# nyu-systems/CLM-GS

Hardware: AMD Instinct MI355X
Metric: training images/s (Rubble-4K 28M Gaussians clm_offload) (higher is better)
Workload: dtype f32

## Files before the change

clm_gs_amd/_lib.py:

```python
import ctypes
import os
import time

import torch

_HERE = os.path.dirname(os.path.abspath(__file__))
LIB_PATH = os.environ.get("CLMGS_LIB_PATH") or os.path.join(_HERE, "libclmgs_hip.so")

_vp, _i, _i64, _f, _sz = ctypes.c_void_p, ctypes.c_int, ctypes.c_int64, ctypes.c_float, ctypes.c_size_t
_d = ctypes.c_double

SIGNATURES = {
    "clmgs_version": (_i, []),
    "clmgs_last_error": (ctypes.c_char_p, []),
    "clmgs_projection_fwd": (_i, [_vp, _i, _i, _vp, _vp, _vp, _vp, _vp, _i, _i, _f, _f, _f, _f, _vp, _vp, _vp, _vp]),
    "clmgs_visibility_select_temp_bytes": (_sz, [_i, _i]),
    "clmgs_visibility_select_count": (_i, [_vp, _i, _i, _vp, _vp, _vp, _vp, _vp, _i, _i, _f, _f, _f, _f, _vp, _sz, _vp]),
    "clmgs_visibility_select_count_blocks": (_i, [_vp, _i, _i, _vp, _vp, _vp, _vp, _vp, _i, _i, _f, _f, _f, _f, _vp, _sz, _vp, _vp]),
    "clmgs_visibility_select_emit": (_i, [_vp, _i, _i, _vp, _vp]),
    "clmgs_visibility_raw": (_i, [_vp, _i, _i, _vp, _vp, _vp, _vp, _vp, _i, _i, _f, _f, _f, _f, _vp]),
    "clmgs_projection_bwd": (_i, [_vp, _i, _i, _vp, _vp, _vp, _vp, _vp, _i, _i, _f, _vp, _vp, _vp, _vp, _vp, _vp, _vp]),
    "clmgs_sh_fwd": (_i, [_vp, _i, _i, _vp, _vp, _vp, _vp]),
    "clmgs_sh_bwd": (_i, [_vp, _i, _i, _vp, _vp, _vp, _vp, _vp, _i, _vp]),
    "clmgs_isect_count_temp_bytes": (_sz, [_i]),
    "clmgs_isect_count": (_i, [_vp, _i, _i, _vp, _vp, _i, _i, _i, _vp, _vp, _vp, _sz]),
    "clmgs_isect_sort_temp_bytes": (_sz, [_i64]),
    "clmgs_isect_emit_sort": (_i, [_vp, _i, _i, _i64, _vp, _vp, _vp, _vp, _i, _i, _i, _vp, _vp, _vp, _sz]),
    "clmgs_isect_offsets": (_i, [_vp, _i64, _vp, _i, _i, _i, _vp]),
    "clmgs_isect2_order_temp_bytes": (_sz, [_i]),
    "clmgs_isect2_order_count": (_i, [_vp, _i, _vp, _vp, _vp, _i, _i, _i, _vp, _vp, _vp, _vp, _vp, _vp, _sz, _vp]),
    "clmgs_isect2_sort_temp_bytes": (_sz, [_i64]),
    "clmgs_isect2_emit_sort": (_i, [_vp, _i, _i64, _vp, _vp, _vp, _vp, _i, _i, _vp, _vp, _vp, _vp, _vp, _sz, _vp]),
    "clmgs_isect2_emit_sort_dev": (_i, [_vp, _i, _i64, _vp, _vp, _vp, _vp, _vp, _i, _i, _vp, _vp, _vp, _vp, _vp, _sz, _vp]),
    "clmgs_isect3_front_temp_bytes": (_sz, [_i, _i]),
    "clmgs_isect3_front": (_i, [_vp, _i, _vp, _vp, _i, _i, _i, _vp, _vp, _vp, _vp, _sz]),
    "clmgs_isect3_bin_temp_bytes": (_sz, [_i64, _i]),
    "clmgs_isect3_bin": (_i, [_vp, _i, _i64, _vp, _i, _i, _vp, _vp, _vp, _vp, _vp, _vp, _vp, _sz]),
    "clmgs_isect3_bin_dev": (_i, [_vp, _i, _i64, _vp, _vp, _i, _i, _vp, _vp, _vp, _vp, _vp, _vp, _vp, _sz]),
    "clmgs_rasterize_fwd_dev": (_i, [_vp, _i, _i, _i64, _vp, _vp, _i, _i, _i, _i, _i, _vp, _vp, _vp, _vp, _vp, _vp]),
    "clmgs_rasterize_bwd_dev": (_i, [_vp, _i, _i, _i64, _vp, _vp, _vp, _i, _i, _i, _i, _i, _vp, _vp, _vp, _vp, _vp, _vp, _vp, _vp, _vp]),
    "clmgs_rasterize_pack_bytes": (_sz, [_i, _i]),
    "clmgs_rasterize_fwd": (_i, [_vp, _i, _i, _i64, _vp, _vp, _vp, _vp, _vp, _i, _i, _i, _i, _i, _vp, _vp, _vp, _vp, _vp, _vp]),
    "clmgs_rasterize_partials_bytes": (_sz, [_i64]),
    "clmgs_rasterize_bwd": (_i, [_vp, _i, _i, _i64, _vp, _vp, _i, _i, _i, _i, _i, _vp, _vp, _vp, _vp, _vp, _vp, _vp, _vp, _vp, _vp, _vp, _vp, _vp, _vp]),
    "clmgs_rasterize4_fwd": (_i, [_vp, _i, _i, _i64, _vp, _vp, _vp, _vp, _vp, _i, _i, _i, _i, _i, _vp, _vp, _vp, _vp, _vp, _vp]),
    "clmgs_rasterize4_bwd": (_i, [_vp, _i, _i, _i64, _vp, _vp, _i, _i, _i, _i, _i, _vp, _vp, _vp, _vp, _vp, _vp, _vp, _vp, _vp, _vp, _vp, _vp, _vp, _vp]),
    "clmgs_rasterize4_slot_bwd": (_i, [_vp, _i, _i, _i64, _vp, _vp, _i, _i, _i, _i, _i, _vp, _vp, _vp, _vp, _vp, _vp, _vp, _vp, _vp, _vp, _vp, _vp, _vp, _vp]),
    "clmgs_rasterize4_fwd_dev": (_i, [_vp, _i, _i, _i64, _vp, _vp, _i, _i, _i, _i, _i, _vp, _vp, _vp, _vp, _vp, _vp]),
    "clmgs_rasterize4_bwd_dev": (_i, [_vp, _i, _i, _i64, _vp, _vp, _vp, _i, _i, _i, _i, _i, _vp, _vp, _vp, _vp, _vp, _vp, _vp, _vp, _vp]),
    "clmgs_preprocess_fwd": (_i, [_vp, _i, _vp, _vp, _vp, _vp, _vp, _vp, _i, _vp, _vp, _vp, _i, _i, _i, _f, _f, _f, _f, _vp, _vp, _vp, _vp, _vp, _vp, _vp, _vp]),
    "clmgs_preprocess_bwd": (_i, [_vp, _i, _vp, _vp, _vp, _vp, _vp, _vp, _i, _vp, _vp, _vp, _i, _i, _i, _f, _vp, _vp, _vp, _vp, _vp, _vp, _vp, _vp, _vp, _vp, _vp, _i, _vp, _vp, _vp, _vp, _i]),
    "clmgs_rasterize_abs_bwd": (_i, [_vp, _i, _i, _i64, _vp, _vp, _i, _i, _i, _i, _i, _vp, _vp, _vp, _vp, _vp, _vp, _vp, _vp, _vp, _vp, _vp, _vp, _vp, _vp, _vp]),
    "clmgs_rasterize_abs_bwd_dev": (_i, [_vp, _i, _i, _i64, _vp, _vp, _vp, _i, _i, _i, _i, _i, _vp, _vp, _vp, _vp, _vp, _vp, _vp, _vp, _vp]),
    "clmgs_preprocess_abs_bwd": (_i, [_vp, _i, _vp, _vp, _vp, _vp, _vp, _vp, _i, _vp, _vp, _vp, _i, _i, _i, _f, _vp, _vp, _vp, _vp, _vp, _vp, _vp, _vp, _vp, _vp, _vp, _i, _vp, _vp, _vp, _vp, _i, _vp]),
    "clmgs_projection_aa_fwd": (_i, [_vp, _i, _i, _vp, _vp, _vp, _vp, _vp, _i, _i, _f, _f, _f, _f, _vp, _vp, _vp, _vp, _vp]),
    "clmgs_projection_aa_bwd": (_i, [_vp, _i, _i, _vp, _vp, _vp, _vp, _vp, _i, _i, _f, _vp, _vp, _vp, _vp, _vp, _vp, _vp, _vp]),
    "clmgs_preprocess_aa_fwd": (_i, [_vp, _i, _vp, _vp, _vp, _vp, _vp, _vp, _i, _vp, _vp, _vp, _i, _i, _i, _f, _f, _f, _f, _vp, _vp, _vp, _vp, _vp, _vp, _vp, _vp]),
    "clmgs_preprocess_aa_bwd": (_i, [_vp, _i, _vp, _vp, _vp, _vp, _vp, _vp, _i, _vp, _vp, _vp, _i, _i, _i, _f, _vp, _vp, _vp, _vp, _vp, _vp, _vp, _vp, _vp, _vp, _vp, _i, _vp, _vp, _vp, _vp, _i]),
    "clmgs_preprocess_aa_abs_bwd": (_i, [_vp, _i, _vp, _vp, _vp, _vp, _vp, _vp, _i, _vp, _vp, _vp, _i, _i, _i, _f, _vp, _vp, _vp, _vp, _vp, _vp, _vp, _vp, _vp, _vp, _vp, _i, _vp, _vp, _vp, _vp, _i, _vp]),
    "clmgs_ssim_fwd": (_i, [_vp, _i, _i, _i, _i, _vp, _vp, _vp, _vp, _vp, _vp]),
    "clmgs_ssim_bwd": (_i, [_vp, _i, _i, _i, _i, _vp, _vp, _vp, _f, _vp, _vp, _vp, _vp]),
    "clmgs_loss_slots": (_i, []),
    "clmgs_l1_ssim_loss_fwd": (_i, [_vp, _i, _i, _vp, _i64, _i64, _i64, _vp, _vp, _vp, _vp, _vp]),
    "clmgs_l1_ssim_loss_bwd": (_i, [_vp, _i, _i, _vp, _i64, _i64, _i64, _vp, _vp, _f, _vp, _vp, _vp, _vp]),
    "clmgs_l1_ssim_loss_masked_fwd": (_i, [_vp, _i, _i, _vp, _i64, _i64, _i64, _vp, _vp, _vp, _vp, _vp, _vp]),
    "clmgs_l1_ssim_loss_masked_bwd": (_i, [_vp, _i, _i, _vp, _i64, _i64, _i64, _vp, _vp, _f, _vp, _vp, _vp, _vp, _vp]),
    "clmgs_exposure_partials_rows": (_i, [_i, _i]),
    "clmgs_exposure_fwd": (_i, [_vp, _i, _i, _vp, _i64, _i64, _i64, _vp, _vp, _i64, _i64, _i64]),
    "clmgs_exposure_bwd": (_i, [_vp, _i, _i, _vp, _i64, _i64, _i64, _vp, _vp, _i64, _i64, _i64, _vp, _i64, _i64, _i64, _vp]),
    "clmgs_exposure_grad_finish": (_i, [_vp, _i, _vp, _vp]),
    "clmgs_invdepth_partials_rows": (_i, [_i, _i]),
    "clmgs_invdepth_pack": (_i, [_vp, _i, _vp, _vp, _vp]),
    "clmgs_invdepth_l1_fwd_bwd": (_i, [_vp, _i, _i, _vp, _i64, _i64, _vp, _f, _f, _vp, _f, _vp, _i64, _i64, _vp]),
    "clmgs_invdepth_finish": (_i, [_vp, _i, _vp, _vp]),
    "clmgs_invdepth_rows_bwd": (_i, [_vp, _i, _vp, _vp, _vp, _vp, _vp, _vp, _vp, _vp, _i]),
    "clmgs_mcmc_relocation": (_i, [_vp, _i64, _vp, _vp, _vp, _vp, _vp]),
    "clmgs_mcmc_reg_grad": (_i, [_vp, _i64, _vp, _i64, _vp, _i64, _vp, _i64, _vp, _i64, _f, _f]),
    "clmgs_mcmc_noise": (_i, [_vp, _i64, _vp, _vp, _vp, _vp, _vp, _f, _vp]),
    "clmgs_rows_gather": (_i, [_vp, _vp, _vp, _vp, _vp, _i, _i64, _i, _i]),
    "clmgs_rows_scatter_add": (_i, [_vp, _vp, _vp, _vp, _vp, _i, _i64, _i, _i]),
    "clmgs_scatter_to_bit": (_i, [_vp, _vp, _i, _vp, _i64, _i]),
    "clmgs_extract_ffs": (_i, [_vp, _vp, _i, _i64, _vp]),
    "clmgs_pair_overlap_count": (_i, [_vp, _vp, _i, _i64, _i, _vp]),
    "clmgs_set_signal": (_i, [_vp, _vp, _i, ctypes.c_int32]),
    "clmgs_adam_rows": (_i, [_vp, _vp, _vp, _vp, _vp, _vp, _i, _vp, _i64, _i, _vp, _d, _d, _d, _i, _i, _f, _i]),
    "clmgs_pack_small": (_i, [_vp, _i64, _vp, _vp, _vp, _vp, _vp]),
    "clmgs_adam_small_packed": (_i, [_vp, _i64, _vp, _vp, _vp, _vp, _vp, _vp, _d, _d, _d, _i, _i, _f, _vp, _i]),
    "clmgs_adam_catch_up": (_i, [_vp, _vp, _vp, _vp, _vp, _vp, _i, _i64, _i, _vp, _d, _d, _d, _i, _i, _i, _vp, _vp, _f, _i]),
    "clmgs_host_adam_rows": (_i, [_vp, _vp, _vp, _vp, _vp, _i64, _i, _vp, _d, _d, _d, _i, _i, _f, _i, _vp, _i]),
    "clmgs_host_pool_start": (_i, [_i]),
    "clmgs_host_usable_cpus": (_i, []),
    "clmgs_memcpy_async": (_i, [_vp, _vp, _vp, _sz, _i]),
    "clmgs_host_rows_prepare": (_i, [_vp, _vp, _vp, _vp, _vp, _vp, _vp, _i64, _i, _vp, _d, _d, _d, _i, _i, _i, _f, _i, _vp, _i]),
    "clmgs_densify_stats": (_i, [_vp, _i64, _vp, _vp, _vp, _i, _f, _f, _vp, _vp, _vp]),
    "clmgs_morton_order_temp_bytes": (_sz, [_i64]),
    "clmgs_morton_order": (_i, [_vp, _i64, _vp, _vp, _vp, _vp, _sz]),
    "clmgs_tsp_tour": (_i, [_i, _vp, _vp]),
    "clmgs_knn3_mean_dist2": (_i, [_vp, _i, _vp, _vp, _f, _f, _f, _f, _i, _i, _i, _i, _vp]),
    "clmgs_host_groups_temp_bytes": (_sz, [_i64]),
    "clmgs_host_groups": (_i, [_vp, _i64, _vp, _vp, _i, _i, _vp, _i, _vp, _vp, _vp, _vp, _vp, _sz]),
    "clmgs_publish_pack": (_i, [_vp, _vp, _vp, _vp, _vp, _i, _i64, _i64, _i64, _i]),
    "clmgs_visibility_candidates": (_i, [_vp, _i, _i, _i, _i, _vp, _vp, _vp, _vp, _i, _i, _f, _f, _f, _f, _f, _vp]),
    "clmgs_small_rows_scatter": (_i, [_vp, _i64, _vp, _vp, _vp, _vp, _vp, _vp, _vp]),
    "clmgs_adam_small_packed_range": (_i, [_vp, _i64, _i64, _i64, _vp, _vp, _vp, _vp, _vp, _vp, _d, _d, _d, _i, _i, _f, _vp, _i]),
    "clmgs_small_deferred_kmax": (_i, []),
    "clmgs_adam_small_deferred": (_i, [_vp, _i64, _vp, _vp, _vp, _vp, _vp, _vp, _vp, _i, _i, _vp, _vp, _vp, _vp, _d, _d, _d,
                                       _f, _i, _vp, _vp, _i, _i, _f, _f, _f, _i, _vp]),
    "clmgs_device_errors": (_i, [_vp, _i]),
    "clmgs_pinned_alloc": (_vp, [_sz]),
    "clmgs_pinned_free": (_i, [_vp]),
}

_lib = None

TIMING = None
STATS = {"n_isects": [], "n_emitted": [], "host_wait_s": 0.0}


class ClmgsError(RuntimeError):
    pass


class _Entry:

    def __init__(self, name, fn, takes_stream):
        self.name, self.fn, self.takes_stream = name, fn, takes_stream

    def __call__(self, *args):
        if TIMING is None or not self.takes_stream:
            return self.fn(*args)
        s, e = torch.cuda.Event(enable_timing=True), torch.cuda.Event(enable_timing=True)
        h = getattr(args[0], "value", args[0])
        st = torch.cuda.ExternalStream(h) if h else torch.cuda.current_stream()
        s.record(st)
        rc = self.fn(*args)
        e.record(st)
        TIMING.setdefault(self.name, []).append((s, e))
        return rc


class _Namespace:
    pass


_NO_STREAM = {"clmgs_version", "clmgs_loss_slots", "clmgs_exposure_partials_rows", "clmgs_invdepth_partials_rows", "clmgs_small_deferred_kmax", "clmgs_isect3_front_temp_bytes",
              "clmgs_isect3_bin_temp_bytes", "clmgs_last_error", "clmgs_isect_count_temp_bytes",
              "clmgs_isect_sort_temp_bytes", "clmgs_host_groups_temp_bytes", "clmgs_isect2_order_temp_bytes", "clmgs_isect2_sort_temp_bytes", "clmgs_visibility_select_temp_bytes", "clmgs_rasterize_pack_bytes", "clmgs_rasterize_partials_bytes", "clmgs_host_adam_rows", "clmgs_host_pool_start", "clmgs_host_usable_cpus", "clmgs_host_rows_prepare", "clmgs_tsp_tour",
              "clmgs_pinned_alloc", "clmgs_pinned_free", "clmgs_device_errors"}


def timing_summary():
    out = {}
    for name, evs in (TIMING or {}).items():
        out[name] = (len(evs), sum(s.elapsed_time(e) for s, e in evs))
    return out


def lib():
    global _lib
    if _lib is None:
        if not os.path.exists(LIB_PATH):
            raise ClmgsError(
                f"{LIB_PATH} not found: build it with `python -c 'import __graft_entry__ as g; g.build()'` "
                "(make -C clm_gs_amd/csrc).  clm_gs_amd has no CPU/eager fallback."
            )
        l = ctypes.CDLL(LIB_PATH)
        ns = _Namespace()
        for name, (res, args) in SIGNATURES.items():
            fn = getattr(l, name)
            fn.restype = res
            fn.argtypes = args
            setattr(ns, name, _Entry(name, fn, name not in _NO_STREAM))
        _lib = ns
    return _lib


def check(rc):
    if rc != 0:
        msg = lib().clmgs_last_error()
        raise ClmgsError(f"libclmgs_hip error {rc}: {msg.decode() if msg else ''}")


def check_device_errors():
    bits = ctypes.c_uint32(0)
    check(lib().clmgs_device_errors(ctypes.byref(bits), 1))
    if bits.value & 4:
        raise ClmgsError("deferred small-attribute Adam: a block of rows was further behind than the recorded step history "
                         "(clmgs_adam_small_deferred, device error bit 4): its parameters are wrong")
    if bits.value:
        raise ClmgsError(f"device error word {bits.value}: no kernel of this library raises that value (4 is the only one "
# ... 68 lines not shown
```

clm_gs_amd/csrc/clm_ops.hip:

```cpp
#include <stdlib.h>

#include "common.h"
#include "vis_math.h"
#include "radix.h"

namespace clmgs {
__device__ uint32_t g_dev_err;
static uint32_t* device_error_word() {
  static thread_local uint32_t* p[16] = {nullptr};
  int dev = 0;
  if (hipGetDevice(&dev) != hipSuccess || dev < 0 || dev >= 16) dev = 0;
  if (!p[dev]) {
    void* a = nullptr;
    if (hipGetSymbolAddress(&a, HIP_SYMBOL(g_dev_err)) == hipSuccess) p[dev] = (uint32_t*)a;
  }
  return p[dev];
}


template <typename IdxT>
__device__ __forceinline__ int64_t row_of(const void* idx, int64_t i) {
  return idx ? (int64_t)reinterpret_cast<const IdxT*>(idx)[i] : i;
}

// ... 426 lines not shown
        int row[4];
#pragma unroll
        for (int k = 0; k < 4; ++k) {
          row[k] = (i + k) / w;
          gg[k] = sg[row[k] * 12 + co + (i + k - row[k] * w)] * grad_scale;
        }
        step(ti, row, pp, mm, vv, gg);
#pragma unroll
        for (int k = 0; k < 4; ++k) sp[row[k] * 12 + co + (i + k - row[k] * w)] = pp[k];
        *reinterpret_cast<float4*>(P + i) = make_float4(pp[0], pp[1], pp[2], pp[3]);
        *reinterpret_cast<float4*>(M + i) = make_float4(mm[0], mm[1], mm[2], mm[3]);
        *reinterpret_cast<float4*>(V + i) = make_float4(vv[0], vv[1], vv[2], vv[3]);
      } else {
        for (int idx = i; idx < n_el; ++idx) {
          const int row[1] = {idx / w};
          float pp[1] = {P[idx]}, mm[1] = {M[idx]}, vv[1] = {V[idx]};
          const float gg[1] = {sg[row[0] * 12 + co + (idx - row[0] * w)] * grad_scale};
          step(ti, row, pp, mm, vv, gg);
          P[idx] = pp[0]; M[idx] = mm[0]; V[idx] = vv[0];
          sp[row[0] * 12 + co + (idx - row[0] * w)] = pp[0];
        }
      }
    }
  }
  __syncthreads();
}

template <bool RANGE>
__global__ void __launch_bounds__(SA_ROWS)
adam_small_packed_kernel(int64_t n, int64_t row_begin, int64_t row_end, SmallAdam t, float4* __restrict__ packed_p,
                         float4* __restrict__ packed_g, float beta1, float beta2, float ob1,
                         float ob2, float eps, float inv_bc1, float inv_sqrt_bc2, float grad_scale,
                         const int32_t* __restrict__ g_stamp, int cur_step) {
  __shared__ __attribute__((aligned(16))) float sg[SA_ROWS * 12];
  __shared__ __attribute__((aligned(16))) float sp[SA_ROWS * 12];
  const int tid = threadIdx.x;
  const int64_t n_blocks = RANGE ? (row_end + SA_ROWS - 1) / SA_ROWS : (n + SA_ROWS - 1) / SA_ROWS;
  for (int64_t blk = (RANGE ? row_begin / SA_ROWS : 0) + blockIdx.x; blk < n_blocks; blk += gridDim.x) {
    const int64_t row0 = blk * SA_ROWS;
    const int rows = (int)min((int64_t)SA_ROWS, n - row0);
    __syncthreads();
    if (g_stamp) {
      __shared__ uint8_t has_g[SA_ROWS];
      if (tid < rows) has_g[tid] = (uint8_t)(g_stamp[row0 + tid] == cur_step);
      __syncthreads();
      small_stage(sg, packed_g, row0, rows, [&](int row) { return has_g[row] != 0; });
    } else {
      small_stage(sg, packed_g, row0, rows, [](int) { return true; });
    }
    small_walk(t, row0, rows, sg, sp, grad_scale,
               [&](int ti, const auto& row, auto& pp, auto& mm, auto& vv, const auto& gg) {
      const float lr_bc = t.lr[ti] * inv_bc1;
      constexpr int N = (int)(sizeof(pp) / sizeof(float));
      float pn[N], m2[N], v2[N];
#pragma unroll
      for (int k = 0; k < N; ++k) {
        m2[k] = mm[k]; v2[k] = vv[k];
        pn[k] = adam_elem(m2[k], v2[k], pp[k], gg[k], lr_bc, beta1, beta2, ob1, ob2, eps, inv_sqrt_bc2);
      }
#pragma unroll
      for (int k = 0; k < N; ++k) {
        const bool act = !RANGE || (row0 + row[k] >= row_begin && row0 + row[k] < row_end);
        pp[k] = act ? pn[k] : pp[k]; mm[k] = act ? m2[k] : mm[k]; vv[k] = act ? v2[k] : vv[k];
      }
    });
    const float4 z = make_float4(0.f, 0.f, 0.f, 0.f);
    for (int i = tid; i < rows * 3; i += SA_ROWS) {
      packed_p[row0 * 3 + i] = reinterpret_cast<const float4*>(sp)[i];
      const float4 gq = reinterpret_cast<const float4*>(sg)[i];
      if (!g_stamp && (gq.x != 0.f || gq.y != 0.f || gq.z != 0.f || gq.w != 0.f))
        packed_g[row0 * 3 + i] = z;
    }
  }
}

constexpr int SD_KMAX = 16;
struct SmallDeferred {
  float lr[SD_KMAX][4];
  float inv_bc1[SD_KMAX], inv_sqrt_bc2[SD_KMAX];
  float pos_margin[SD_KMAX + 1], scale_gain[SD_KMAX + 1];
  int to_step;
};

__global__ void __launch_bounds__(SA_ROWS)
adam_small_deferred_kernel(int64_t n, SmallAdam t, float4* __restrict__ packed_p, const float4* __restrict__ packed_g,
                           const int32_t* __restrict__ g_stamp, int32_t* __restrict__ blk_last, SmallDeferred d,
                           float beta1, float beta2, float ob1, float ob2, float eps, float grad_scale, int C,
                           const float* __restrict__ viewmats, const float* __restrict__ Ks, float W, float H, float eps2d,
                           float near_plane, float far_plane, int flush_all, uint8_t* __restrict__ blk_flag, int n_hist,
                           uint32_t* __restrict__ dev_err) {
  __shared__ __attribute__((aligned(16))) float sg[SA_ROWS * 12];
  __shared__ __attribute__((aligned(16))) float sp[SA_ROWS * 12];
  __shared__ int gstep_s[SA_ROWS];
  __shared__ float cam_s[VB_MAX_CAMS][VB_CAM_F];
  const int tid = threadIdx.x;
  if (!flush_all) {
    for (int c = tid; c < C; c += SA_ROWS) vis_store_cam(cam_s[c], viewmats + 16 * c, Ks + 9 * c, W, H);
  }
  const float near_m = near_plane - (fabsf(near_plane) * 1e-5f + 1e-6f);
  const float far_m = far_plane + fabsf(far_plane) * 1e-5f;
  const int64_t n_blocks = (n + SA_ROWS - 1) / SA_ROWS;
  for (int64_t blk = blockIdx.x; blk < n_blocks; blk += gridDim.x) {
    const int last = blk_last[blk];
    int k = d.to_step - last;
    if (k <= 0 && (flush_all || !blk_flag)) continue;
    if (k > n_hist) {
      if (tid == 0 && dev_err) atomicOr(dev_err, 4u);
      k = n_hist;
    }
    const int64_t row0 = blk * SA_ROWS;
    const int rows = (int)min((int64_t)SA_ROWS, n - row0);
    __syncthreads();
    if (!flush_all) {
      const int kk = min(max(k, 0), SD_KMAX);
      bool cand = false;
      if (tid < rows) {
        const float* x = t.p[0] + 3 * (row0 + tid);
        const float* ls = t.p[2] + 3 * (row0 + tid);
        const float m[3] = {x[0], x[1], x[2]};
        const float sgn = __expf(fmaxf(ls[0], fmaxf(ls[1], ls[2]))) * d.scale_gain[kk];
        const float smax2g = sgn * sgn;
        cand = !(smax2g < 1e30f);
        for (int c = 0; c < C && !cand; ++c)
          cand = vis_candidate(lds_cam(cam_s[c]), cam_s[c][16], m, smax2g, d.pos_margin[kk], W, H, eps2d, near_m, far_m);
      }
      const bool any = __syncthreads_or(cand);
      if (blk_flag && tid == 0) blk_flag[blk] = any ? 1 : 0;
      if (k <= 0 || (!any && k < SD_KMAX)) continue;
    }
    if (tid < rows) {
      const int gs = g_stamp[row0 + tid];
      gstep_s[tid] = (gs > last && gs <= d.to_step) ? gs : -1;
    }
    __syncthreads();
    small_stage(sg, packed_g, row0, rows, [&](int row) { return gstep_s[row] >= 0; });
    small_walk(t, row0, rows, sg, sp, grad_scale,
               [&](int ti, const auto& row, auto& pp, auto& mm, auto& vv, const auto& gg) {
      constexpr int N = (int)(sizeof(pp) / sizeof(float));
      int gst[N];
#pragma unroll
      for (int q = 0; q < N; ++q) gst[q] = gstep_s[row[q]];
      for (int s_ = last + 1; s_ <= d.to_step; ++s_) {
        const int j = d.to_step - s_;
        const float lr_bc = d.lr[j][ti] * d.inv_bc1[j];
        const float isb2 = d.inv_sqrt_bc2[j];
#pragma unroll
        for (int q = 0; q < N; ++q)
          pp[q] = adam_elem(mm[q], vv[q], pp[q], gst[q] == s_ ? gg[q] : 0.f, lr_bc, beta1, beta2, ob1, ob2, eps, isb2);
      }
    });
    for (int i = tid; i < rows * 3; i += SA_ROWS) packed_p[row0 * 3 + i] = reinterpret_cast<const float4*>(sp)[i];
    if (tid == 0) blk_last[blk] = d.to_step;
  }
}

__global__ void __launch_bounds__(256)
pack_small_kernel(int64_t n, const float* __restrict__ xyz, const float* __restrict__ opa,
                  const float* __restrict__ sca, const float* __restrict__ rot,
                  float4* __restrict__ packed_p) {
  for (int64_t r = blockIdx.x * (int64_t)blockDim.x + threadIdx.x; r < n;
       r += (int64_t)gridDim.x * blockDim.x) {
    const float4 q = *reinterpret_cast<const float4*>(rot + 4 * r);
    packed_p[3 * r] = make_float4(xyz[3 * r], xyz[3 * r + 1], xyz[3 * r + 2], opa[r]);
    packed_p[3 * r + 1] = make_float4(sca[3 * r], sca[3 * r + 1], sca[3 * r + 2], q.x);
    packed_p[3 * r + 2] = make_float4(q.y, q.z, q.w, 0.f);
  }
}

__global__ void __launch_bounds__(256)
small_rows_scatter_kernel(int64_t n_rows, const int64_t* __restrict__ rows, const float4* __restrict__ src,
                          float* __restrict__ xyz, float* __restrict__ opa, float* __restrict__ sca,
                          float* __restrict__ rot, float4* __restrict__ packed_p) {
  for (int64_t i = blockIdx.x * (int64_t)blockDim.x + threadIdx.x; i < n_rows;
       i += (int64_t)gridDim.x * blockDim.x) {
    const int64_t r = rows[i];
    const float4 a = src[3 * i], b = src[3 * i + 1], c = src[3 * i + 2];
    xyz[3 * r] = a.x; xyz[3 * r + 1] = a.y; xyz[3 * r + 2] = a.z;
    opa[r] = a.w;
    sca[3 * r] = b.x; sca[3 * r + 1] = b.y; sca[3 * r + 2] = b.z;
    *reinterpret_cast<float4*>(rot + 4 * r) = make_float4(b.w, c.x, c.y, c.z);
    packed_p[3 * r] = a; packed_p[3 * r + 1] = b; packed_p[3 * r + 2] = make_float4(c.x, c.y, c.z, 0.f);
  }
}

__global__ void __launch_bounds__(256)
densify_stats_kernel(int64_t n, const int64_t* __restrict__ filter,
                     const float* __restrict__ v_means2d, const int32_t* __restrict__ radii,
                     int only_visible, float half_w, float half_h, float* __restrict__ max_radii2D,
                     float* __restrict__ accum, float* __restrict__ denom) {
  for (int64_t i = blockIdx.x * (int64_t)blockDim.x + threadIdx.x; i < n;
       i += (int64_t)gridDim.x * blockDim.x) {
    const int r = radii[i];
    if (only_visible && r <= 0) continue;
    const int64_t g = filter ? filter[i] : i;
    const float gx = v_means2d[2 * i] * half_w, gy = v_means2d[2 * i + 1] * half_h;
    max_radii2D[g] = fmaxf(max_radii2D[g], (float)r);
    accum[g] += sqrtf(gx * gx + gy * gy);
    denom[g] += 1.f;
  }
}

}

using namespace clmgs;

extern "C" int clmgs_rows_gather(void* stream, float* dst, const float* src, const void* dst_idx,
                                 const void* src_idx, int idx_is_64, int64_t n_rows, int cols,
                                 int grid_blocks) {
  return rows_move<false>(stream, dst, src, dst_idx, src_idx, idx_is_64, n_rows, cols, grid_blocks);
}

extern "C" int clmgs_publish_pack(void* stream, float* msg, const float* table, const int64_t* own_rows,
                                  const int32_t* stamp, int step, int64_t lo, int64_t n_rows, int64_t chunk,
                                  int cols) {
  CLMGS_CHECK_ARG(n_rows >= 0 && chunk >= n_rows && cols > 0 && cols % 4 == 0);
  if (n_rows == 0) return 0;
  CLMGS_CHECK_ARG(msg && table && own_rows && (((uintptr_t)msg | (uintptr_t)table) & 15) == 0);
  const int64_t total = n_rows * (cols / 4);
  hipLaunchKernelGGL(publish_pack_kernel, dim3(min(ceil_div(total, 256), 256 * 8)), dim3(256), 0, (hipStream_t)stream,
                     msg, table, own_rows, stamp, step, lo, n_rows, chunk, cols / 4);
  CLMGS_LAUNCH_CHECK();
  return 0;
}

extern "C" int clmgs_rows_scatter_add(void* stream, float* dst, const float* src,
                                      const void* dst_idx, const void* src_idx, int idx_is_64,
                                      int64_t n_rows, int cols, int grid_blocks) {
  return rows_move<true>(stream, dst, src, dst_idx, src_idx, idx_is_64, n_rows, cols, grid_blocks);
}

#define DISPATCH_ELEM(bytes, CALL)                    \
  switch (bytes) {                                    \
    case 1: { typedef int8_t T; CALL; } break;        \
    case 2: { typedef int16_t T; CALL; } break;       \
    case 4: { typedef int32_t T; CALL; } break;       \
// ... 224 lines not shown
                     (float)(1.0 - beta1), (float)(1.0 - beta2), keep_grad)
  if (idx_is_64) { if (v4) CLMGS_CATCH_UP(int64_t, 4); else CLMGS_CATCH_UP(int64_t, 1); }
  else { if (v4) CLMGS_CATCH_UP(int32_t, 4); else CLMGS_CATCH_UP(int32_t, 1); }
#undef CLMGS_CATCH_UP
  CLMGS_LAUNCH_CHECK();
  return 0;
}

extern "C" int clmgs_pack_small(void* stream, int64_t n, const float* xyz, const float* opacity,
                                const float* scaling, const float* rotation, void* packed_p) {
  CLMGS_CHECK_ARG(n >= 0);
  if (n == 0) return 0;
  CLMGS_CHECK_ARG(xyz && opacity && scaling && rotation && packed_p && (((uintptr_t)packed_p & 15) == 0));
  hipLaunchKernelGGL(pack_small_kernel, dim3(min(ceil_div(n, 256), 256 * 16)), dim3(256), 0,
                     (hipStream_t)stream, n, xyz, opacity, scaling, rotation, (float4*)packed_p);
  CLMGS_LAUNCH_CHECK();
  return 0;
}

extern "C" int clmgs_small_rows_scatter(void* stream, int64_t n_rows, const int64_t* rows, const void* lines,
                                        float* xyz, float* opacity, float* scaling, float* rotation,
                                        void* packed_p) {
  CLMGS_CHECK_ARG(n_rows >= 0);
  if (n_rows == 0) return 0;
  CLMGS_CHECK_ARG(rows && lines && xyz && opacity && scaling && rotation && packed_p &&
                  (((uintptr_t)packed_p | (uintptr_t)lines | (uintptr_t)rotation) & 15) == 0);
  hipLaunchKernelGGL(small_rows_scatter_kernel, dim3(min(ceil_div(n_rows, 256), 256 * 16)), dim3(256), 0,
                     (hipStream_t)stream, n_rows, rows, (const float4*)lines, xyz, opacity, scaling, rotation,
                     (float4*)packed_p);
  CLMGS_LAUNCH_CHECK();
  return 0;
}

extern "C" int clmgs_adam_small_packed_range(void* stream, int64_t n, int64_t row_begin, int64_t row_end,
                                             float* const* params, float* const* exp_avg,
                                             float* const* exp_avg_sq, const double* lr4, void* packed_p,
                                             void* packed_g, double beta1, double beta2, double eps, int step,
                                             int bias_correction, float grad_scale, const int32_t* g_stamp,
                                             int cur_step);

extern "C" int clmgs_adam_small_packed(void* stream, int64_t n, float* const* params,
                                       float* const* exp_avg, float* const* exp_avg_sq,
                                       const double* lr4, void* packed_p, void* packed_g,
                                       double beta1, double beta2, double eps, int step,
                                       int bias_correction, float grad_scale, const int32_t* g_stamp,
                                       int cur_step) {
  return clmgs_adam_small_packed_range(stream, n, 0, -1, params, exp_avg, exp_avg_sq, lr4, packed_p, packed_g, beta1,
                                       beta2, eps, step, bias_correction, grad_scale, g_stamp, cur_step);
}

extern "C" int clmgs_adam_small_packed_range(void* stream, int64_t n, int64_t row_begin, int64_t row_end,
                                             float* const* params, float* const* exp_avg,
                                             float* const* exp_avg_sq, const double* lr4, void* packed_p,
                                             void* packed_g, double beta1, double beta2, double eps, int step,
                                             int bias_correction, float grad_scale, const int32_t* g_stamp,
                                             int cur_step) {
  CLMGS_CHECK_ARG(n >= 0 && step >= 1);
  const bool ranged = row_end >= 0;
  if (ranged) CLMGS_CHECK_ARG(row_begin >= 0 && row_begin <= row_end && row_end <= n);
  if (n == 0 || (ranged && row_end == row_begin)) return 0;
  CLMGS_CHECK_ARG(lr4 && packed_p && packed_g && (((uintptr_t)packed_p | (uintptr_t)packed_g) & 15) == 0);
  SmallAdam t;
  CLMGS_CHECK_ARG(small_adam_fill(&t, params, exp_avg, exp_avg_sq, lr4));
  float inv_bc1, inv_sqrt_bc2;
  adam_bias_host(beta1, beta2, step, bias_correction, &inv_bc1, &inv_sqrt_bc2);
  const float ob1 = (float)(1.0 - beta1), ob2 = (float)(1.0 - beta2);
  if (ranged) {
    const int64_t blocks = (row_end + SA_ROWS - 1) / SA_ROWS - row_begin / SA_ROWS;
    hipLaunchKernelGGL(adam_small_packed_kernel<true>, dim3(min(blocks, (int64_t)256 * 16)), dim3(SA_ROWS), 0,
                       (hipStream_t)stream, n, row_begin, row_end, t, (float4*)packed_p, (float4*)packed_g,
                       (float)beta1, (float)beta2, ob1, ob2, (float)eps, inv_bc1, inv_sqrt_bc2, grad_scale, g_stamp,
                       cur_step);
  } else {
    hipLaunchKernelGGL(adam_small_packed_kernel<false>, dim3(min(ceil_div(n, SA_ROWS), 256 * 16)), dim3(SA_ROWS), 0,
                       (hipStream_t)stream, n, (int64_t)0, n, t, (float4*)packed_p, (float4*)packed_g, (float)beta1,
                       (float)beta2, ob1, ob2, (float)eps, inv_bc1, inv_sqrt_bc2, grad_scale, g_stamp, cur_step);
  }
  CLMGS_LAUNCH_CHECK();
  return 0;
}

extern "C" int clmgs_small_deferred_kmax(void) { return SD_KMAX; }

extern "C" int clmgs_adam_small_deferred(void* stream, int64_t n, float* const* params, float* const* exp_avg,
                                         float* const* exp_avg_sq, void* packed_p, const void* packed_g,
                                         const int32_t* g_stamp, int32_t* blk_last, int to_step, int n_hist,
                                         const double* lr4_hist, const int32_t* step_index, const float* pos_margin,
                                         const float* scale_gain, double beta1, double beta2, double eps,
                                         float grad_scale, int C, const float* viewmats, const float* Ks, int width,
                                         int height, float eps2d, float near_plane, float far_plane, int flush_all,
                                         uint8_t* blk_flag) {
  CLMGS_CHECK_ARG(n >= 0 && to_step >= 0 && n_hist >= 0 && n_hist <= SD_KMAX);
  CLMGS_CHECK_ARG(!blk_flag || !flush_all);
  if (n == 0) return 0;
  if (n_hist == 0) {
    if (blk_flag) CLMGS_HIP(hipMemsetAsync(blk_flag, 1, (size_t)((n + SA_ROWS - 1) / SA_ROWS), (hipStream_t)stream));
    return 0;
  }
  CLMGS_CHECK_ARG(packed_p && packed_g && g_stamp && blk_last && lr4_hist && step_index && pos_margin && scale_gain &&
                  (((uintptr_t)packed_p | (uintptr_t)packed_g) & 15) == 0);
  CLMGS_CHECK_ARG(flush_all || (C >= 1 && C <= VB_MAX_CAMS && viewmats && Ks && width > 0 && height > 0));
  SmallAdam t;
  CLMGS_CHECK_ARG(small_adam_fill(&t, params, exp_avg, exp_avg_sq, nullptr));
  SmallDeferred d;
  for (int j = 0; j < SD_KMAX; ++j) {
    const int jj = j < n_hist ? j : n_hist - 1;
    for (int i = 0; i < 4; ++i) d.lr[j][i] = (float)lr4_hist[4 * jj + i];
    CLMGS_CHECK_ARG(step_index[jj] >= 1);
    adam_bias_host(beta1, beta2, step_index[jj], 1, &d.inv_bc1[j], &d.inv_sqrt_bc2[j]);
  }
  for (int k = 0; k <= SD_KMAX; ++k) {
    const int kk = k <= n_hist ? k : n_hist;
    d.pos_margin[k] = pos_margin[kk];
    d.scale_gain[k] = scale_gain[kk];
  }
  d.to_step = to_step;
  const float ob1 = (float)(1.0 - beta1), ob2 = (float)(1.0 - beta2);
  hipLaunchKernelGGL(adam_small_deferred_kernel, dim3(min(ceil_div(n, SA_ROWS), 256 * 16)), dim3(SA_ROWS), 0,
                     (hipStream_t)stream, n, t, (float4*)packed_p, (const float4*)packed_g, g_stamp, blk_last, d,
                     (float)beta1, (float)beta2, ob1, ob2, (float)eps, grad_scale, C, viewmats, Ks, (float)width,
                     (float)height, eps2d, near_plane, far_plane, flush_all, blk_flag, n_hist, device_error_word());
  CLMGS_LAUNCH_CHECK();
  return 0;
}

extern "C" int clmgs_device_errors(uint32_t* out, int reset) {
  CLMGS_CHECK_ARG(out);
  CLMGS_HIP(hipDeviceSynchronize());
  CLMGS_HIP(hipMemcpyFromSymbol(out, HIP_SYMBOL(clmgs::g_dev_err), sizeof(uint32_t)));
  if (reset && *out) {
    const uint32_t z = 0;
    CLMGS_HIP(hipMemcpyToSymbol(HIP_SYMBOL(clmgs::g_dev_err), &z, sizeof(z)));
  }
  return 0;
}

extern "C" int clmgs_densify_stats(void* stream, int64_t n, const int64_t* filter,
                                   const float* v_means2d, const int32_t* radii,
                                   int only_visible, float half_w, float half_h,
                                   float* max_radii2D, float* xyz_gradient_accum,
                                   float* denom) {
  CLMGS_CHECK_ARG(n >= 0);
  if (n == 0) return 0;
  CLMGS_CHECK_ARG(v_means2d && radii && max_radii2D && xyz_gradient_accum && denom);
  const int grid = min(ceil_div(n, 256), 256 * 8);
  hipLaunchKernelGGL(densify_stats_kernel, dim3(grid), dim3(256), 0, (hipStream_t)stream, n, filter,
                     v_means2d, radii, only_visible, half_w, half_h, max_radii2D,
                     xyz_gradient_accum, denom);
  CLMGS_LAUNCH_CHECK();
  return 0;
}
```

clm_gs_amd/csrc/isect.hip:

```cpp
#include <stdlib.h>

#include "common.h"
#include "gs_math.h"
#include "radix.h"
#include "vis_math.h"
#include "isect_math.h"

namespace clmgs {

__global__ void __launch_bounds__(256)
isect_count_kernel(int64_t CN, const float* __restrict__ means2d, const int32_t* __restrict__ radii,
                   float tile_size, int tile_w, int tile_h, int32_t* __restrict__ tiles_per_gauss,
                   int64_t* __restrict__ cum) {
  for (int64_t i = blockIdx.x * (int64_t)blockDim.x + threadIdx.x; i < CN;
       i += (int64_t)gridDim.x * blockDim.x) {
    int cnt = 0;
    const int r = radii[i];
    if (r > 0) {
      const float2 m = *reinterpret_cast<const float2*>(means2d + 2 * i);
      const TileBox b = tile_box(m.x, m.y, (float)r, tile_size, tile_w, tile_h);
      cnt = (b.x1 - b.x0) * (b.y1 - b.y0);
    }
    tiles_per_gauss[i] = cnt;
    cum[i] = cnt;
// ... 431 lines not shown
}

extern "C" size_t clmgs_isect2_sort_temp_bytes(int64_t n_isects) {
  if (n_isects <= 0) return 256;
  return 6 * align_up((size_t)n_isects * 4, 256) + radix_table_bytes(n_isects) + 256;
}

static int isect2_emit_sort_impl(void* stream, int V, int64_t n_isects, const float* depths,
                                 const int32_t* order, const int64_t* cum,
                                 const uint64_t* boxes, int tile_width, int tile_height,
                                 int32_t* flatten_ids, int32_t* offsets, int64_t* isect_ids,
                                 int32_t* emit_slot, void* temp, size_t temp_bytes,
                                 const int64_t* row_cum, const int64_t* n_dev) {
  CLMGS_CHECK_ARG(V >= 0 && n_isects >= 0 && offsets);
  hipStream_t s = (hipStream_t)stream;
  const int n_tiles = tile_width * tile_height;
  if (n_isects == 0) {
    CLMGS_HIP(hipMemsetAsync(offsets, 0, sizeof(int32_t) * (size_t)n_tiles, s));
    return 0;
  }
  CLMGS_CHECK_ARG(n_isects < ((int64_t)1 << 31));
  CLMGS_CHECK_ARG(depths && order && cum && boxes && flatten_ids && temp);
  CLMGS_CHECK_ARG(temp_bytes >= clmgs_isect2_sort_temp_bytes(n_isects));
  char* base = (char*)temp;
  const size_t a4 = align_up((size_t)n_isects * 4, 256);
  uint32_t* k_a = (uint32_t*)base; base += a4;
  uint32_t* k_b = (uint32_t*)base; base += a4;
  char* v_a = base; base += 2 * a4;
  char* v_b = base; base += 2 * a4;
  uint32_t* table = (uint32_t*)base;
  const bool slots = emit_slot != nullptr;
  CLMGS_CHECK_ARG(!slots || row_cum);
  const int tile_bits = ilog2_floor((unsigned)n_tiles) + 1;
  const int n_blocks = (int)((n_isects + RS_MIN_CHUNK - 1) / RS_MIN_CHUNK);
  if (slots)
    hipLaunchKernelGGL((isect2_emit_hist_kernel<true>), dim3(n_blocks), dim3(256), 0, s, V, n_isects, n_dev, order,
                       (const unsigned long long*)boxes, cum, tile_width, row_cum, k_a, (int32_t*)nullptr, (int2*)v_a,
                       n_blocks, table);
  else
    hipLaunchKernelGGL((isect2_emit_hist_kernel<false>), dim3(n_blocks), dim3(256), 0, s, V, n_isects, n_dev, order,
                       (const unsigned long long*)boxes, cum, tile_width, row_cum, k_a, (int32_t*)v_a, (int2*)nullptr,
                       n_blocks, table);
  CLMGS_LAUNCH_CHECK();
  uint32_t* sorted = nullptr;
  int rc;
  if (slots)
    rc = radix_sort_pairs_impl<uint32_t, int2, RS_DEFAULT_ITEMS>(s, n_isects, k_a, k_b, (int2*)v_a, (int2*)v_b, (int2*)nullptr,
                                                                  0, tile_bits, table, &sorted, n_dev, flatten_ids, emit_slot,
                                                                  true);
  else
    rc = radix_sort_pairs_impl<uint32_t, int32_t, RS_DEFAULT_ITEMS>(s, n_isects, k_a, k_b, (int32_t*)v_a, (int32_t*)v_b,
                                                                     flatten_ids, 0, tile_bits, table, &sorted, n_dev,
                                                                     nullptr, nullptr, true);
  if (rc) return rc;
  hipLaunchKernelGGL(isect2_offsets_kernel, dim3(min(ceil_div(n_isects, 256), 256 * 16)), dim3(256), 0, s,
                     n_isects, sorted, n_tiles, offsets, flatten_ids, depths, isect_ids, n_dev);
  CLMGS_LAUNCH_CHECK();
  return 0;
}

extern "C" int clmgs_isect2_emit_sort(void* stream, int V, int64_t n_isects, const float* depths,
                                      const int32_t* order, const int64_t* cum,
                                      const uint64_t* boxes, int tile_width, int tile_height,
                                      int32_t* flatten_ids, int32_t* offsets, int64_t* isect_ids,
                                      int32_t* emit_slot, void* temp, size_t temp_bytes,
                                      const int64_t* row_cum) {
  return isect2_emit_sort_impl(stream, V, n_isects, depths, order, cum, boxes, tile_width, tile_height,
                               flatten_ids, offsets, isect_ids, emit_slot, temp, temp_bytes, row_cum, nullptr);
}

extern "C" int clmgs_isect2_emit_sort_dev(void* stream, int V, int64_t capacity, const int64_t* n_isects_dev,
                                          const float* depths, const int32_t* order, const int64_t* cum,
                                          const uint64_t* boxes, int tile_width, int tile_height,
                                          int32_t* flatten_ids, int32_t* offsets, int64_t* isect_ids,
                                          int32_t* emit_slot, void* temp, size_t temp_bytes,
                                          const int64_t* row_cum) {
  CLMGS_CHECK_ARG(n_isects_dev && capacity > 0);
  return isect2_emit_sort_impl(stream, V, capacity, depths, order, cum, boxes, tile_width, tile_height,
                               flatten_ids, offsets, isect_ids, emit_slot, temp, temp_bytes, row_cum, n_isects_dev);
}

namespace clmgs {

constexpr int VB_CH = 4;

__device__ __forceinline__ int vis_classify(const Cam& c, float kc, const float m[3], float smax2,
                                            float W, float H, float eps2d, float near_m, float far_m,
                                            float near_p, float far_p, bool accept_ok) {
  const float x = c.R[0] * m[0] + c.R[1] * m[1] + c.R[2] * m[2] + c.t[0];
  const float y = c.R[3] * m[0] + c.R[4] * m[1] + c.R[5] * m[2] + c.t[1];
  const float z = c.R[6] * m[0] + c.R[7] * m[1] + c.R[8] * m[2] + c.t[2];
  if (z < near_m || z > far_m) return 0;
  const float rz = __builtin_amdgcn_rcpf(z);
  const float mx = c.fx * x * rz + c.cx, my = c.fy * y * rz + c.cy;
  const float B = smax2 * rz * rz * kc + eps2d;
  if (accept_ok && z > near_p && z < far_p && B < 400.f && mx >= 1.f && mx <= W - 1.f && my >= 1.f &&
      my <= H - 1.f)
    return 1;
  const float Rb = 3.03f * __builtin_amdgcn_sqrtf(2.f * B + 0.1f) + 2.f;
  return (mx + Rb <= 0.f || mx - Rb >= W || my + Rb <= 0.f || my - Rb >= H) ? 0 : 2;
}

__global__ void __launch_bounds__(256)
visibility_bits_kernel(int C, int N, int W64, const float* __restrict__ means,
                       const float* __restrict__ quats_raw, const float* __restrict__ log_scales,
                       const float* __restrict__ viewmats, const float* __restrict__ Ks, float W, float H,
                       float eps2d, float near_plane, float far_plane, float radius_clip,
                       unsigned long long* __restrict__ bits, int64_t* __restrict__ counts,
                       const uint8_t* __restrict__ blk_flag) {
  __shared__ float cam_s[VB_MAX_CAMS][VB_CAM_F];
  __shared__ float row_s[256][10];
  __shared__ unsigned short cand[256 * VB_CH];
  __shared__ int n_cand;
  __shared__ unsigned long long wb[VB_CH][4];
  __shared__ unsigned long long anyw[4];
  const int tid = threadIdx.x, lane = tid & 63;
  const unsigned long long lt = (1ull << lane) - 1ull;
  const float near_m = near_plane - (fabsf(near_plane) * 1e-5f + 1e-6f);
  const float far_m = far_plane + fabsf(far_plane) * 1e-5f;
  const float near_p = near_plane + (fabsf(near_plane) * 1e-5f + 1e-6f);
  const float far_p = far_plane - fabsf(far_plane) * 1e-5f;
  const bool accept_ok = radius_clip < 1.5f && eps2d >= 0.3f;
  const int wid = tid >> 6;
  for (int c = tid; c < C; c += 256) {
    const Cam cam = load_cam(viewmats + 16 * c, Ks + 9 * c);
    float* f = cam_s[c];
    for (int i = 0; i < 9; ++i) f[i] = cam.R[i];
    f[9] = cam.t[0]; f[10] = cam.t[1]; f[11] = cam.t[2];
    f[12] = cam.fx; f[13] = cam.fy; f[14] = cam.cx; f[15] = cam.cy;
    f[16] = vis_cam_kc(cam, W, H);
  }
  const int n_rb = (W64 + 3) / 4;
  float nm0 = 0.f, nm1 = 0.f, nm2 = 0.f, nl0 = 0.f, nl1 = 0.f, nl2 = 0.f;
  float4 nq = make_float4(0.f, 0.f, 0.f, 0.f);
  auto fetch = [&](int rbn) {
    const int n = rbn * 256 + tid;
    const bool live_n = rbn < n_rb && (!blk_flag || blk_flag[rbn]);
    const int nn = (live_n && n < N) ? n : 0;
    nm0 = means[3 * nn]; nm1 = means[3 * nn + 1]; nm2 = means[3 * nn + 2];
    nq = *reinterpret_cast<const float4*>(quats_raw + 4 * nn);
    nl0 = log_scales[3 * nn]; nl1 = log_scales[3 * nn + 1]; nl2 = log_scales[3 * nn + 2];
  };
  fetch(blockIdx.x);
  for (int rb = blockIdx.x; rb < n_rb; rb += gridDim.x) {
    const int n = rb * 256 + tid;
    const bool in = n < N;
    const float m[3] = {nm0, nm1, nm2};
    const float4 q4 = nq;
    const float s0 = __expf(nl0), s1 = __expf(nl1), s2 = __expf(nl2);
    fetch(rb + gridDim.x);
    if (blk_flag && !blk_flag[rb]) {
      if (tid < (C + 1) * 4) {
        const int c = tid >> 2, w = rb * 4 + (tid & 3);
        if (w < W64) { bits[(size_t)c * W64 + w] = 0ull; counts[(size_t)c * W64 + w] = 0; }
      }
      for (int q = tid + 256; q < (C + 1) * 4; q += 256) {
        const int c = q >> 2, w = rb * 4 + (q & 3);
        if (w < W64) { bits[(size_t)c * W64 + w] = 0ull; counts[(size_t)c * W64 + w] = 0; }
      }
      continue;
    }
    const float smax = fmaxf(s0, fmaxf(s1, s2));
    const float smax2 = smax * smax;
    const float qn2 = q4.x * q4.x + q4.y * q4.y + q4.z * q4.z + q4.w * q4.w;
    const bool row_ok = accept_ok && qn2 >= 1e-20f && qn2 <= 1e20f && (s0 + s1 + s2) < 1e30f;
    lds_barrier();
    {
      float* r = row_s[tid];
      r[0] = m[0]; r[1] = m[1]; r[2] = m[2]; r[3] = q4.x; r[4] = q4.y; r[5] = q4.z; r[6] = q4.w;
      r[7] = s0; r[8] = s1; r[9] = s2;
    }
    if (tid < 4) anyw[tid] = 0ull;
    for (int c0 = 0; c0 < C; c0 += VB_CH) {
      const int cn = min(VB_CH, C - c0);
      if (tid < VB_CH * 4) wb[tid >> 2][tid & 3] = 0ull;
      if (tid == 0) n_cand = 0;
      lds_barrier();
      for (int cc = 0; cc < cn; ++cc) {
        const Cam cam = load_cam(viewmats + 16 * (c0 + cc), Ks + 9 * (c0 + cc));
        const int cls = in ? vis_classify(cam, cam_s[c0 + cc][16], m, smax2, W, H, eps2d, near_m, far_m,
                                          near_p, far_p, row_ok) : 0;
        const unsigned long long acc = __ballot(cls == 1);
        if (lane == 0 && acc) atomicOr(&wb[cc][wid], acc);
        const bool pass = cls == 2;
        const unsigned long long b = __ballot(pass);
        int base = 0;
        if (lane == 0 && b) base = atomicAdd(&n_cand, __popcll(b));
        base = __builtin_amdgcn_readfirstlane(base);
        if (pass) cand[base + __popcll(b & lt)] = (unsigned short)(tid | (cc << 8));
      }
      lds_barrier();
      const int nc = n_cand;
      for (int k = tid; k < nc; k += 256) {
        const int e = cand[k], r = e & 255, cc = e >> 8;
        const Cam cam = lds_cam(cam_s[c0 + cc]);
        const float* rr = row_s[r];
        const float mm[3] = {rr[0], rr[1], rr[2]};
        const float qq[4] = {rr[3], rr[4], rr[5], rr[6]};
        const float ss[3] = {rr[7], rr[8], rr[9]};
        const Proj p = project_fwd(cam, mm, qq, ss, W, H, eps2d, near_plane, far_plane, radius_clip);
        if (p.radius > 0) atomicOr(&wb[cc][r >> 6], 1ull << (r & 63));
      }
      lds_barrier();
      if (tid < cn * 4) {
        const int cc = tid >> 2, j = tid & 3, w = rb * 4 + j;
        if (w < W64) {
          const unsigned long long b = wb[cc][j];
          bits[(size_t)(c0 + cc) * W64 + w] = b;
          counts[(size_t)(c0 + cc) * W64 + w] = __popcll(b);
          if (b) atomicOr(&anyw[j], b);
        }
      }
    }
    lds_barrier();
    if (tid < 4 && rb * 4 + tid < W64) {
      bits[(size_t)C * W64 + rb * 4 + tid] = anyw[tid];
      counts[(size_t)C * W64 + rb * 4 + tid] = __popcll(anyw[tid]);
    }
  }
}

__global__ void __launch_bounds__(256)
visibility_candidates_kernel(int C, int N, int own_lo, int own_hi, const float* __restrict__ means,
                             const float* __restrict__ log_scales, const float* __restrict__ viewmats,
                             const float* __restrict__ Ks, float W, float H, float eps2d, float near_plane,
                             float far_plane, float pos_margin, float scale_gain, uint8_t* __restrict__ mask) {
  __shared__ float cam_s[VB_MAX_CAMS][VB_CAM_F];
  const int tid = threadIdx.x;
  for (int c = tid; c < C; c += 256) {
    const Cam cam = load_cam(viewmats + 16 * c, Ks + 9 * c);
    float* f = cam_s[c];
    for (int i = 0; i < 9; ++i) f[i] = cam.R[i];
    f[9] = cam.t[0]; f[10] = cam.t[1]; f[11] = cam.t[2];
    f[12] = cam.fx; f[13] = cam.fy; f[14] = cam.cx; f[15] = cam.cy;
    f[16] = vis_cam_kc(cam, W, H);
  }
  __syncthreads();
  const float near_m = near_plane - (fabsf(near_plane) * 1e-5f + 1e-6f);
  const float far_m = far_plane + fabsf(far_plane) * 1e-5f;
  for (int n = blockIdx.x * 256 + tid; n < N; n += gridDim.x * 256) {
    if (n >= own_lo && n < own_hi) {
      mask[n] = 0;
      continue;
    }
    const float m[3] = {means[3 * n], means[3 * n + 1], means[3 * n + 2]};
    const float lmax = fmaxf(log_scales[3 * n], fmaxf(log_scales[3 * n + 1], log_scales[3 * n + 2]));
    const float sg = __expf(lmax) * scale_gain;
    const float smax2g = sg * sg;
    bool any = !(smax2g < 1e30f);
    for (int c = 0; c < C && !any; ++c)
      any = vis_candidate(lds_cam(cam_s[c]), cam_s[c][16], m, smax2g, pos_margin, W, H, eps2d, near_m, far_m);
    mask[n] = any ? 1 : 0;
  }
}

__global__ void __launch_bounds__(256)
visibility_emit_kernel(int C, int N, int W64, const unsigned long long* __restrict__ bits,
                       const int64_t* __restrict__ scan, int64_t* __restrict__ out) {
  const int64_t total = (int64_t)(C + 1) * W64 * 64;
  for (int64_t t = blockIdx.x * (int64_t)blockDim.x + threadIdx.x; t < total;
       t += (int64_t)gridDim.x * blockDim.x) {
    const int64_t word = t >> 6;
    const int bit = (int)(t & 63);
    const unsigned long long b = bits[word];
    if ((b >> bit) & 1ull) {
      const int64_t end = scan[word];
      const int64_t pos = end - __popcll(b) + __popcll(b & ((1ull << bit) - 1ull));
      const int w = (int)(word % W64);
      out[pos] = (int64_t)w * 64 + bit;
    }
  }
}

}

extern "C" size_t clmgs_visibility_select_temp_bytes(int C, int N) {
  const size_t words = (size_t)(C + 1) * (size_t)((N + 63) / 64);
  return 2 * align_up(words * 8, 256) + scan_scratch_bytes((int64_t)words) + 256;
}

extern "C" int clmgs_visibility_select_count_blocks(void* stream, int C, int N, const float* means,
                                                    const float* quats_raw, const float* log_scales,
                                                    const float* viewmats, const float* Ks, int width, int height,
                                                    float eps2d, float near_plane, float far_plane,
                                                    float radius_clip, void* temp, size_t temp_bytes,
                                                    int64_t* cum_totals, const uint8_t* block_flags);

extern "C" int clmgs_visibility_select_count(void* stream, int C, int N, const float* means,
                                             const float* quats_raw, const float* log_scales,
                                             const float* viewmats, const float* Ks, int width,
                                             int height, float eps2d, float near_plane,
                                             float far_plane, float radius_clip, void* temp,
                                             size_t temp_bytes, int64_t* cum_totals) {
  return clmgs_visibility_select_count_blocks(stream, C, N, means, quats_raw, log_scales, viewmats, Ks, width, height,
                                              eps2d, near_plane, far_plane, radius_clip, temp, temp_bytes, cum_totals,
                                              nullptr);
}

extern "C" int clmgs_visibility_select_count_blocks(void* stream, int C, int N, const float* means,
                                                    const float* quats_raw, const float* log_scales,
                                                    const float* viewmats, const float* Ks, int width, int height,
                                                    float eps2d, float near_plane, float far_plane,
                                                    float radius_clip, void* temp, size_t temp_bytes,
                                                    int64_t* cum_totals, const uint8_t* block_flags) {
  CLMGS_CHECK_ARG(C >= 1 && C <= 64 && N >= 1 && width > 0 && height > 0);
  CLMGS_CHECK_ARG(means && quats_raw && log_scales && viewmats && Ks && temp && cum_totals);
  CLMGS_CHECK_ARG(temp_bytes >= clmgs_visibility_select_temp_bytes(C, N));
  hipStream_t s = (hipStream_t)stream;
  const int W64 = (N + 63) / 64;
  const size_t words = (size_t)(C + 1) * W64;
  char* base = (char*)temp;
  unsigned long long* bits = (unsigned long long*)base; base += align_up(words * 8, 256);
  int64_t* counts = (int64_t*)base; base += align_up(words * 8, 256);
  int64_t* scratch = (int64_t*)base;
  hipLaunchKernelGGL(visibility_bits_kernel, dim3(min(ceil_div((int64_t)W64 * 64, 256), 256 * 8)),
                     dim3(256), 0, s, C, N, W64, means, quats_raw, log_scales, viewmats, Ks,
                     (float)width, (float)height, eps2d, near_plane, far_plane, radius_clip, bits, counts, block_flags);
  CLMGS_LAUNCH_CHECK();
  const int rc = inclusive_scan_i64(s, (int64_t)words, counts, scratch);
  if (rc) return rc;
  for (int r = 0; r <= C; ++r)
    CLMGS_HIP(hipMemcpyAsync(cum_totals + r, counts + (size_t)(r + 1) * W64 - 1, sizeof(int64_t),
                             hipMemcpyDeviceToDevice, s));
  return 0;
}

extern "C" int clmgs_visibility_select_emit(void* stream, int C, int N, const void* temp,
                                            int64_t* out) {
  CLMGS_CHECK_ARG(C >= 1 && N >= 1 && temp && out);
  const int W64 = (N + 63) / 64;
  const size_t words = (size_t)(C + 1) * W64;
  const char* base = (const char*)temp;
  const unsigned long long* bits = (const unsigned long long*)base; base += align_up(words * 8, 256);
  const int64_t* scan = (const int64_t*)base;
  hipLaunchKernelGGL(visibility_emit_kernel, dim3(min(ceil_div((int64_t)words * 64, 256), 256 * 32)),
                     dim3(256), 0, (hipStream_t)stream, C, N, W64, bits, scan, out);
  CLMGS_LAUNCH_CHECK();
  return 0;
}


extern "C" int clmgs_visibility_candidates(void* stream, int C, int N, int own_lo, int own_hi, const float* means,
                                           const float* log_scales, const float* viewmats, const float* Ks,
                                           int width, int height, float eps2d, float near_plane, float far_plane,
                                           float pos_margin, float scale_gain, uint8_t* mask) {
  CLMGS_CHECK_ARG(C >= 1 && C <= 64 && N >= 1 && width > 0 && height > 0);
  CLMGS_CHECK_ARG(means && log_scales && viewmats && Ks && mask);
  CLMGS_CHECK_ARG(pos_margin >= 0.f && scale_gain >= 1.f && own_lo >= 0 && own_hi >= own_lo);
  hipLaunchKernelGGL(visibility_candidates_kernel, dim3(min(ceil_div((int64_t)N, 256), 256 * 16)), dim3(256), 0,
                     (hipStream_t)stream, C, N, own_lo, own_hi, means, log_scales, viewmats, Ks, (float)width,
                     (float)height, eps2d, near_plane, far_plane, pos_margin, scale_gain, mask);
  CLMGS_LAUNCH_CHECK();
  return 0;
}
```

clm_gs_amd/csrc/vis_math.h:

```cpp
#pragma once
#include "common.h"
#include "gs_math.h"

namespace clmgs {

constexpr int VB_CAM_F = 20;
constexpr int VB_MAX_CAMS = 64;

__device__ __forceinline__ float vis_cam_kc(const Cam& c, float W, float H) {
  const float tan_fovx = 0.5f * W / c.fx, tan_fovy = 0.5f * H / c.fy;
  const float limx = fmaxf(fabsf((W - c.cx) / c.fx), fabsf(c.cx / c.fx)) + 0.3f * tan_fovx;
  const float limy = fmaxf(fabsf((H - c.cy) / c.fy), fabsf(c.cy / c.fy)) + 0.3f * tan_fovy;
  return 0.505f * (c.fx * c.fx * (1.f + limx * limx) + c.fy * c.fy * (1.f + limy * limy));
}

__device__ __forceinline__ Cam lds_cam(const float* f) {
  Cam c;
#pragma unroll
  for (int i = 0; i < 9; ++i) c.R[i] = f[i];
  c.t[0] = f[9]; c.t[1] = f[10]; c.t[2] = f[11];
  c.fx = f[12]; c.fy = f[13]; c.cx = f[14]; c.cy = f[15];
  return c;
}


__device__ __forceinline__ bool vis_candidate(const Cam& c, float kc, const float m[3], float smax2g, float d,
                                              float W, float H, float eps2d, float near_m, float far_m) {
  const float x = c.R[0] * m[0] + c.R[1] * m[1] + c.R[2] * m[2] + c.t[0];
  const float y = c.R[3] * m[0] + c.R[4] * m[1] + c.R[5] * m[2] + c.t[1];
  const float z = c.R[6] * m[0] + c.R[7] * m[1] + c.R[8] * m[2] + c.t[2];
  const float zl = z - d, zh = z + d;
  if (zh < near_m || zl > far_m) return false;
  const float zc = fmaxf(fmaxf(zl, near_m), 1e-12f), zf = fmaxf(fminf(zh, far_m), zc);
  const float rzc = 1.f / zc, rzf = 1.f / zf;
  const float xh = x + d, xl = x - d, yh = y + d, yl = y - d;
  const float tx_max = xh > 0.f ? xh * rzc : xh * rzf, tx_min = xl < 0.f ? xl * rzc : xl * rzf;
  const float ty_max = yh > 0.f ? yh * rzc : yh * rzf, ty_min = yl < 0.f ? yl * rzc : yl * rzf;
  const float B = smax2g * rzc * rzc * kc + eps2d;
  const float Rb = 1.001f * (3.03f * sqrtf(2.f * B + 0.1f) + 2.f) + 1.f;
  const float mx_max = c.fx * tx_max + c.cx, mx_min = c.fx * tx_min + c.cx;
  const float my_max = c.fy * ty_max + c.cy, my_min = c.fy * ty_min + c.cy;
  return !(mx_max + Rb <= 0.f || mx_min - Rb >= W || my_max + Rb <= 0.f || my_min - Rb >= H);
}


__device__ __forceinline__ void vis_store_cam(float* f, const float* viewmat, const float* K, float W, float H) {
  const Cam cam = load_cam(viewmat, K);
  for (int i = 0; i < 9; ++i) f[i] = cam.R[i];
  f[9] = cam.t[0]; f[10] = cam.t[1]; f[11] = cam.t[2];
  f[12] = cam.fx; f[13] = cam.fy; f[14] = cam.cx; f[15] = cam.cy;
  f[16] = vis_cam_kc(cam, W, H);
}

}
```

clm_gs_amd/gsplat.py:

```python

import time

import torch

from . import _lib
from ._lib import check, dptr, stream

F32, I32, I64 = torch.float32, torch.int32, torch.int64


class _Projection(torch.autograd.Function):
    @staticmethod
    def forward(ctx, means, quats, scales, viewmats, Ks, width, height, eps2d, near_plane,
                far_plane, radius_clip):
        L = _lib.lib()
        means, quats, scales = means.contiguous(), quats.contiguous(), scales.contiguous()
        viewmats, Ks = viewmats.contiguous(), Ks.contiguous()
        C, N = viewmats.shape[0], means.shape[0]
        dev = means.device
        radii = torch.empty((C, N), dtype=I32, device=dev)
        means2d = torch.empty((C, N, 2), dtype=F32, device=dev)
        depths = torch.empty((C, N), dtype=F32, device=dev)
        conics = torch.empty((C, N, 3), dtype=F32, device=dev)
        check(L.clmgs_projection_fwd(
# ... 50 lines not shown
            float(near_plane), float(far_plane), float(radius_clip), dptr(radii), dptr(means2d),
            dptr(depths), dptr(conics), dptr(comps)))
        ctx.save_for_backward(means, quats, scales, viewmats, Ks, radii)
        ctx.cfg = (int(width), int(height), float(eps2d))
        ctx.mark_non_differentiable(radii)
        return radii, means2d, depths, conics, comps

    @staticmethod
    def backward(ctx, _v_radii, v_means2d, v_depths, v_conics, v_comps):
        L = _lib.lib()
        means, quats, scales, viewmats, Ks, radii = ctx.saved_tensors
        width, height, eps2d = ctx.cfg
        C, N = radii.shape
        dev = means.device
        if v_means2d is None:
            v_means2d = torch.zeros((C, N, 2), dtype=F32, device=dev)
        if v_conics is None:
            v_conics = torch.zeros((C, N, 3), dtype=F32, device=dev)
        v_means2d, v_conics = v_means2d.contiguous(), v_conics.contiguous()
        v_depths = v_depths.contiguous() if v_depths is not None else None
        v_comps = v_comps.contiguous() if v_comps is not None else None
        v_means = torch.empty_like(means)
        v_quats = torch.empty_like(quats)
        v_scales = torch.empty_like(scales)
        check(L.clmgs_projection_aa_bwd(
            stream(), C, N, dptr(means), dptr(quats), dptr(scales), dptr(viewmats), dptr(Ks),
            width, height, eps2d, dptr(radii), dptr(v_means2d, F32), dptr(v_depths, F32, True),
            dptr(v_conics, F32), dptr(v_comps, F32, True), dptr(v_means), dptr(v_quats), dptr(v_scales)))
        return v_means, v_quats, v_scales, None, None, None, None, None, None, None, None


def fully_fused_projection(means, covars, quats, scales, viewmats, Ks, width, height, eps2d=0.3,
                           near_plane=0.01, far_plane=1e10, radius_clip=0.0, packed=False,
                           sparse_grad=False, calc_compensations=False):
    if covars is not None:
        raise NotImplementedError("the CLM-GS engines always pass covars=None")
    if calc_compensations:
        if not packed:
            return _ProjectionAA.apply(means, quats, scales, viewmats, Ks, width, height, eps2d, near_plane,
                                       far_plane, radius_clip)
        with torch.no_grad():
            radii, means2d, depths, conics, comps = _ProjectionAA.apply(
                means, quats, scales, viewmats, Ks, width, height, eps2d, near_plane, far_plane, radius_clip)
            camera_ids, gaussian_ids = torch.nonzero(radii > 0, as_tuple=True)
            return (camera_ids, gaussian_ids, radii[camera_ids, gaussian_ids],
                    means2d[camera_ids, gaussian_ids], depths[camera_ids, gaussian_ids],
                    conics[camera_ids, gaussian_ids], comps[camera_ids, gaussian_ids])
    if not packed:
        radii, means2d, depths, conics = _Projection.apply(
            means, quats, scales, viewmats, Ks, width, height, eps2d, near_plane, far_plane,
            radius_clip)
        return radii, means2d, depths, conics, None
    with torch.no_grad():
        radii, means2d, depths, conics = _Projection.apply(
            means, quats, scales, viewmats, Ks, width, height, eps2d, near_plane, far_plane,
            radius_clip)
        camera_ids, gaussian_ids = torch.nonzero(radii > 0, as_tuple=True)
        return (camera_ids, gaussian_ids, radii[camera_ids, gaussian_ids],
                means2d[camera_ids, gaussian_ids], depths[camera_ids, gaussian_ids],
                conics[camera_ids, gaussian_ids], None)


def visibility_radii(means, quats, scales, viewmats, Ks, width, height, eps2d=0.3,
                     near_plane=0.01, far_plane=1e10, radius_clip=0.0, raw=False):
    L = _lib.lib()
    means, quats, scales = means.contiguous(), quats.contiguous(), scales.contiguous()
    viewmats, Ks = viewmats.contiguous(), Ks.contiguous()
    C, N = viewmats.shape[0], means.shape[0]
    radii = torch.empty((C, N), dtype=I32, device=means.device)
    if raw:
        check(L.clmgs_visibility_raw(
            stream(), C, N, dptr(means, F32), dptr(quats, F32), dptr(scales, F32), dptr(viewmats, F32),
            dptr(Ks, F32), int(width), int(height), float(eps2d), float(near_plane), float(far_plane),
            float(radius_clip), dptr(radii)))
        return radii
    check(L.clmgs_projection_fwd(
        stream(), C, N, dptr(means, F32), dptr(quats, F32), dptr(scales, F32), dptr(viewmats, F32),
        dptr(Ks, F32), int(width), int(height), float(eps2d), float(near_plane), float(far_plane),
        float(radius_clip), dptr(radii), None, None, None))
    return radii


def visibility_select(means, quats_raw, log_scales, viewmats, Ks, width, height, eps2d=0.3,
                      near_plane=0.01, far_plane=1e10, radius_clip=0.0, block_flags=None):
    L = _lib.lib()
    means, quats_raw, log_scales = means.contiguous(), quats_raw.contiguous(), log_scales.contiguous()
    viewmats, Ks = viewmats.contiguous(), Ks.contiguous()
    C, N = viewmats.shape[0], means.shape[0]
    dev = means.device
    tb = L.clmgs_visibility_select_temp_bytes(C, N)
    temp = torch.empty((tb,), dtype=torch.uint8, device=dev)
    cum = torch.empty((C + 1,), dtype=I64, device=dev)
    check(L.clmgs_visibility_select_count_blocks(
        stream(), C, N, dptr(means, F32), dptr(quats_raw, F32), dptr(log_scales, F32), dptr(viewmats, F32),
        dptr(Ks, F32), int(width), int(height), float(eps2d), float(near_plane), float(far_plane),
        float(radius_clip), dptr(temp), tb, dptr(cum), dptr(block_flags, torch.uint8, True)))
    _t0 = time.perf_counter()
    ends = cum.tolist()
    _lib.STATS["host_wait_s"] += time.perf_counter() - _t0
    out = torch.empty((max(ends[-1], 1),), dtype=I64, device=dev)
    if ends[-1] > 0:
        check(L.clmgs_visibility_select_emit(stream(), C, N, dptr(temp), dptr(out)))
    starts = [0] + ends[:-1]
    pieces = tuple(out[a:b] for a, b in zip(starts, ends))
    return pieces[:C], pieces[C]


def visibility_candidates(means, log_scales, viewmats, Ks, width, height, pos_margin, scale_gain, own_lo, own_hi,
                          eps2d=0.3, near_plane=0.01, far_plane=1e10):
    L = _lib.lib()
    means, log_scales = means.contiguous(), log_scales.contiguous()
    viewmats, Ks = viewmats.contiguous(), Ks.contiguous()
    C, N = viewmats.shape[0], means.shape[0]
    mask = torch.empty((N,), dtype=torch.uint8, device=means.device)
    check(L.clmgs_visibility_candidates(
        stream(), C, N, int(own_lo), int(own_hi), dptr(means, F32), dptr(log_scales, F32), dptr(viewmats, F32),
        dptr(Ks, F32), int(width), int(height), float(eps2d), float(near_plane), float(far_plane),
        float(pos_margin), float(scale_gain), dptr(mask)))
    return torch.nonzero(mask).flatten()


class _SphericalHarmonics(torch.autograd.Function):
    @staticmethod
    def forward(ctx, degree, dirs, coeffs, masks):
        L = _lib.lib()
        lead = dirs.shape[:-1]
        n = dirs.numel() // 3
        assert coeffs.shape[-2:] == (16, 3) or coeffs.shape[-1] == 48, coeffs.shape
        d2, c2 = dirs.contiguous(), coeffs.contiguous()
        m2 = masks.contiguous().view(torch.uint8) if masks is not None else None
        colors = torch.empty(lead + (3,), dtype=F32, device=dirs.device)
        check(L.clmgs_sh_fwd(stream(), n, int(degree), dptr(d2, F32), dptr(c2, F32),
                             dptr(m2, torch.uint8, True), dptr(colors)))
        ctx.save_for_backward(d2, c2, m2)
        ctx.degree = int(degree)
        ctx.n = n
        return colors

    @staticmethod
    def backward(ctx, v_colors):
        L = _lib.lib()
        d2, c2, m2 = ctx.saved_tensors
        v_colors = v_colors.contiguous()
        v_coeffs = torch.empty_like(c2) if ctx.needs_input_grad[2] else None
        v_dirs = torch.empty_like(d2) if ctx.needs_input_grad[1] else None
        if v_coeffs is None:
            v_coeffs_buf = torch.empty_like(c2)
        else:
            v_coeffs_buf = v_coeffs
        check(L.clmgs_sh_bwd(stream(), ctx.n, ctx.degree, dptr(d2), dptr(c2),
                             dptr(m2, torch.uint8, True), dptr(v_colors, F32), dptr(v_coeffs_buf),
                             0, dptr(v_dirs, F32, True)))
        return None, v_dirs, v_coeffs, None


def spherical_harmonics(degrees_to_use, dirs, coeffs, masks=None):
    return _SphericalHarmonics.apply(degrees_to_use, dirs, coeffs, masks)


@torch.no_grad()
def isect_tiles(means2d, radii, depths, tile_size, tile_width, tile_height, sort=True,
                packed=False, n_cameras=None, camera_ids=None, gaussian_ids=None):
    if packed or not sort:
        raise NotImplementedError("the CLM-GS engines call isect_tiles(packed=False, sort=True)")
    L = _lib.lib()
    C, N = radii.shape
    dev = radii.device
    means2d, radii, depths = means2d.contiguous(), radii.contiguous(), depths.contiguous()
    tiles_per_gauss = torch.empty((C, N), dtype=I32, device=dev)
    cum = torch.empty((C * N,), dtype=I64, device=dev)
    if C * N == 0:
        return tiles_per_gauss, torch.empty(0, dtype=I64, device=dev), torch.empty(0, dtype=I32, device=dev)
    tb = L.clmgs_isect_count_temp_bytes(C * N)
    temp = torch.empty((tb,), dtype=torch.uint8, device=dev)
    check(L.clmgs_isect_count(stream(), C, N, dptr(means2d, F32), dptr(radii, I32), int(tile_size),
                              int(tile_width), int(tile_height), dptr(tiles_per_gauss), dptr(cum),
                              dptr(temp), tb))
    n_isects = int(cum[-1].item())
    _lib.STATS["n_isects"].append(n_isects)
    if len(_lib.STATS["n_isects"]) > 4096:
        del _lib.STATS["n_isects"][:2048]
        del _lib.STATS["n_emitted"][:2048]
    isect_ids = torch.empty((n_isects,), dtype=I64, device=dev)
    flatten_ids = torch.empty((n_isects,), dtype=I32, device=dev)
    if n_isects:
        sb = L.clmgs_isect_sort_temp_bytes(n_isects)
        temp2 = torch.empty((sb,), dtype=torch.uint8, device=dev)
# ... 275 lines not shown
```

clm_gs_amd/strategies/clm_offload/engine.py:

```python
import math
import os

import torch

from ... import _lib, clm_kernels, dp, fast_tsp, mcmc, utils
from ...cameras import camera_loss_mask
from ...clm_kernels import (apply_camera_exposure, camera_depth_term, check_depth_prior_args,
                            send_shs2cpu_grad_buffer_stream, send_shs2gpu_stream, spherical_harmonics_bwd_inplace)
from ...densification import check_mcmc_args, update_densification_stats_offload_accum_grads
from ...gsplat import (fully_fused_projection, isect_offset_encode, isect_tiles,
                       rasterize_to_pixels, spherical_harmonics)
from ...host import pinned_empty
from ..base_engine import (select_filters, TILE_SIZE, calculate_filters, colors_with_depth, pipeline_forward_one_step,
                           split_depth, torch_compiled_loss)

_BITMAP_DTYPE = {4: torch.int8, 8: torch.int8, 16: torch.int16, 32: torch.int32, 64: torch.int64}


def pipeline_forward_one_step_shs_inplace(filtered_opacity_gpu, filtered_scaling_gpu,
                                          filtered_rotation_gpu, filtered_xyz_gpu, filtered_shs,
                                          camera, scene, gaussians, background, pipe_args, render_mode="RGB"):
    viewmat = camera.world_view_transform.transpose(0, 1)
    K = camera.K
    n_selected = filtered_xyz_gpu.shape[0]
# ... 154 lines not shown


def _gpu_adam_step(gaussians, args, visibility_mask, grad_div=None):
    grad_div = float(grad_div or args.bsz)
    small = gaussians.all_parameters()[:4]
    if args.stop_update_param or args.sparse_adam:
        for param in small:
            if param.grad is not None:
                param.grad /= grad_div
        if not args.stop_update_param:
            gaussians.optimizer.gpu_adam.step(visibility=visibility_mask)
        gaussians.optimizer.gpu_adam.zero_grad(set_to_none=True)
        return
    gaussians.optimizer.gpu_step_scaled(1.0 / grad_div)
    gaussians._clean_grad_ptrs = tuple(p.grad.data_ptr() for p in small if p.grad is not None)


def _pipeline_streams(gaussians):
    sts = getattr(gaussians, "_clmgs_streams", None)
    if sts is None:
        try:
            lo, hi = torch.cuda.Stream.priority_range()
        except AttributeError:
            lo, hi = 0, -1
        sts = gaussians._clmgs_streams = {
            "aux": torch.cuda.Stream(),
            "mem": [torch.cuda.Stream(priority=hi) for _ in range(2)],
            "raster": [torch.cuda.Stream(priority=lo) for _ in range(2)]}
    return sts


def reserve_working_set(gaussians, n_cameras_in_flight=2):
    W, H = int(utils.get_img_width()), int(utils.get_img_height())
    P, N = W * H, int(gaussians._xyz.shape[0])
    I = int(1.0 * P)
    V = min(N, max(1, N // 6))
    k = int(n_cameras_in_flight)
    sts = _pipeline_streams(gaussians)
    plan = {
        "front": (sts["mem"][0], k * (20 * P + 70 * I + 96 * V)),
        "mem": (sts["mem"][1], k * 48 * P + (1 << 20)),
        "raster": (sts["raster"][0], 2 * k * 64 * int(0.8 * I)),
        "default": (torch.cuda.current_stream(), 240 * N + 64 * V * 4),
    }
    out = {}
    try:
        free_now = torch.cuda.mem_get_info(gaussians._xyz.device)[0]
    except Exception:
        free_now = None
    total = sum(int(nb) for _, nb in plan.values())
    shrink = 1.0 if not free_now or total <= free_now / 3 else (free_now / 3) / total
    for name, (st, nbytes) in plan.items():
        nbytes = int(nbytes * shrink)
        if nbytes < (1 << 20):
            out[name] = 0
            continue
        try:
            with torch.cuda.stream(st):
                blk = torch.empty((nbytes,), dtype=torch.uint8, device=gaussians._xyz.device)
                small = [torch.empty((1 << 19,), dtype=torch.uint8, device=gaussians._xyz.device) for _ in range(16)]
                del blk, small
            out[name] = nbytes
        except torch.cuda.OutOfMemoryError:
            torch.cuda.empty_cache()
            out[name] = 0
    return out


class _Batch:
    """State of one HBM-resident batch, handed from stage to stage (see _train_one_batch_hbm)."""


def _stage_visibility(b):
    gaussians, args, cams = b.gaussians, b.args, b.cameras
    N = b.N
    b.touched = b.touched_rows = None
    b.small_owner = bool(getattr(gaussians, "small_owner", False) and gaussians.lazy_rows and dp.active()
                         and not args.stop_update_param)
    if b.small_owner:
        with torch.no_grad(), _lib.host_region("dp_small_fetch"), dp.phase("S"):
            gaussians.small_prepare(cams)
    b.small_deferred = bool(getattr(gaussians, "small_deferred", False) and b.fused and gaussians.lazy_rows
                            and not args.stop_update_param and getattr(args, "packed_small", True))
    blk_flags = None
    if b.small_deferred:
        with torch.no_grad():
            blk_flags = gaussians.small_catch_up(cams)
    with torch.no_grad():
        if b.fused:
            with _lib.host_region("select_filters"):
                b.filters, b.touched_rows = select_filters(cams, gaussians._xyz.detach(), gaussians._scaling.detach(),
                                                           gaussians._rotation.detach(), block_flags=blk_flags)
        else:
            b.filters, _, _ = calculate_filters(cams, gaussians.get_xyz, gaussians.get_opacity,
                                                gaussians.get_scaling, gaussians.get_rotation)
    if b.small_owner and os.environ.get("CLMGS_DP_DEBUG") and b.touched_rows is not None:
        lo_, hi_ = dp.owner_range(N)
        foreign = b.touched_rows[(b.touched_rows < lo_) | (b.touched_rows >= hi_)]
        cand_ = getattr(gaussians, "_dbg_cand", None)
        miss = -1
        if cand_ is not None and gaussians._small_since > 0:
            isc = torch.zeros((N,), dtype=torch.bool, device=foreign.device)
            isc[cand_] = True
            miss = int((~isc[foreign]).sum())
        print("DPDEBUG batch rank %d since %d foreign touched rows %d not candidates %d" % (
            dp.rank(), gaussians._small_since, foreign.numel(), miss), flush=True)
        assert miss <= 0
    b.sparsity = [len(f) / float(N) for f in b.filters]
    b.ordered_cams = list(range(b.bsz))
    if getattr(args, "reference_camera_order", False):
        _, b.cameras, b.filters, b.sparsity, b.ordered_cams = order_calculation(
            list(b.filters), list(cams), N, b.bsz, None, args)[:5]


def _stage_plan(b):
    gaussians, args, N, bsz = b.gaussians, b.args, b.N, b.bsz
    b.lazy = gaussians.lazy_rows and not args.stop_update_param
    mode = getattr(args, "overlap_cameras", True)
    b.pipelined = b.fused and mode in (True, "pipeline")
    b.use_packed = (b.fused and getattr(args, "packed_small", True) and not args.sparse_adam
                    and not args.stop_update_param)
    b.locality = bool(b.lazy and dp.active() and getattr(args, "dp_locality", False))
    b.locality_sparse = bool(dp.active() and getattr(args, "dp_locality", False) and args.sparse_adam and b.fused
                             and not args.stop_update_param and not b.lazy)
    if getattr(args, "dp_locality", False) and dp.active():
        assert b.touched_rows is not None and (b.locality_sparse or (b.locality and b.use_packed and gaussians.first_touch_grads)), (
            "dp_locality needs the fused front end and either the dense deferred row optimizer with the packed "
            "small-attribute tables and first-touch gradient stores (defaults) or sparse_adam")
    need_mask = b.touched_rows is None or args.sparse_adam or (dp.active() and not b.locality) or not b.lazy
    if need_mask:
        b.touched = torch.zeros((N,), dtype=torch.bool, device=gaussians._xyz.device)
        if b.touched_rows is not None:
            utils.fill_rows(b.touched, b.touched_rows, True)
        else:
            for f in b.filters:
                utils.fill_rows(b.touched, f, True)
        if dp.active() and not b.locality_sparse:
            b.local_touched = b.touched
            b.touched = dp.allreduce_touched(b.touched)
            b.touched_rows = None
    b.row_adam = gaussians.optimizer.cpu_adam
    b.params = gaussians._parameters
    b.grad_buf = b.parameters_grad_buffer[:N]
    b.params.grad = b.grad_buf
    b.row_adam.global_step += 1
    b.step = b.row_adam.global_step
    _mark_batch(gaussians)
    b.group = b.row_adam.param_groups[0]
    b.st = b.row_adam.state[b.params]
    b.default_stream = torch.cuda.current_stream()
    b.side_event = None
    b.col_lr = b.row_adam._col_lr(b.params.device)
    if b.touched_rows is None:
        b.touched_rows = torch.nonzero(b.touched).flatten()
    b.touched_rows = b.touched_rows.to(torch.int32)
    _lib.STATS.setdefault("touched_rows", []).append(int(b.touched_rows.shape[0]))
    b.ft_stamp = gaussians._row_g_step if (b.lazy and b.fused and gaussians.first_touch_grads) else None


def _mark_batch(gaussians):
    gaussians._lazy_dirty = True
    gaussians._mutations = getattr(gaussians, "_mutations", 0) + 1
    gaussians._sorted_tag = None


def _row_update(b, rows, zero_grad_rows=False):
    clm_kernels.adam_rows(b.params.data, None if zero_grad_rows else b.grad_buf, b.st["exp_avg"],
                          b.st["exp_avg_sq"], rows, b.col_lr,
                          b.group["betas"][0], b.group["betas"][1], b.group["eps"], b.step,
                          b.group["bias_correction"], 1.0 / (b.bsz * dp.world_size()), True)


def _stage_exchange_head(b):
    gaussians, args, N, bsz, step = b.gaussians, b.args, b.N, b.bsz, b.step
    params, touched_rows = b.params, b.touched_rows
    b.owner = b.border = None
    b.split_catch = False
    b.dp_ev_b0 = b.dp_ev_b1 = b.dp_comm = None
    b.dp_split = False
    if b.locality:
        b.dp_split = bool(b.pipelined and bsz >= 2 and getattr(args, "dp_overlap", True))
        with _lib.host_region("dp_border_plan"), dp.phase("plan"):
            b.border = dp.border_plan(touched_rows.long(), N, first_rows=b.filters[0] if b.dp_split else None,
                                      last_rows=b.filters[bsz - 1] if b.dp_split else None,
                                      publish_counts=not b.small_owner)
        gaussians._owner_dirty = True
        own_rows = b.border.own_rows
        if own_rows.numel():
            with dp.phase("catch_up_own"):
                gaussians.catch_up_rows(own_rows.to(torch.int32), to_step=step - 1)
        if b.dp_split:
            b.dp_comm = getattr(gaussians, "_dp_comm_stream", None)
            if b.dp_comm is None:
                b.dp_comm = gaussians._dp_comm_stream = torch.cuda.Stream()
            b.dp_comm.wait_stream(b.default_stream)
            with torch.cuda.stream(b.dp_comm):
                with dp.phase("B0"):
                    dp.border_params_out(params.data, b.border, "params0")
                b.dp_ev_b0 = torch.cuda.Event()
                b.dp_ev_b0.record(b.dp_comm)
                with dp.phase("B1"):
                    dp.border_params_out(params.data, b.border, "params1")
                b.dp_ev_b1 = torch.cuda.Event()
                b.dp_ev_b1.record(b.dp_comm)
        else:
            with dp.phase("B"):
                dp.border_params_out(params.data, b.border)
    elif b.locality_sparse:
        with _lib.host_region("dp_border_plan"), dp.phase("plan"):
            b.border = dp.border_plan(touched_rows.long(), N)
        gaussians._owner_dirty = True
        with dp.phase("B"):
            dp.border_params_out(params.data, b.border)
    elif b.lazy and dp.active() and getattr(args, "dp_owner_computes", False):
        b.owner = dp.owner_plan(touched_rows.long(), N)
        gaussians._owner_dirty = True
        own_rows = touched_rows[b.owner.lo:b.owner.hi]
        if b.owner.hi > b.owner.lo:
            gaussians.catch_up_rows(own_rows, to_step=step - 1)
        dp.owner_gather_rows(params.data, b.owner)
    elif b.lazy:
        if (b.pipelined and bsz >= 2 and getattr(args, "split_catch_up", True) and b.filters is not None):
            b.foreign_rows = None
            if dp.active():
                lt = getattr(b, "local_touched", None)
                assert lt is not None
                b.foreign_rows = touched_rows[~lt[touched_rows.long()]]
            b.split_catch = True
            s_front = _pipeline_streams(gaussians)["mem"][0]
            s_front.wait_stream(b.default_stream)
            b.first_catch_done = bool(getattr(args, "early_first_catch_up", True))
            if b.first_catch_done and b.filters[0].numel():
                with torch.cuda.stream(s_front):
                    gaussians.catch_up_rows(b.filters[0], to_step=step - 1)
        else:
            gaussians.catch_up_rows(touched_rows, to_step=step - 1)
    elif not args.stop_update_param and not args.sparse_adam:
        untouched_rows = torch.nonzero(~b.touched).flatten().to(torch.int32)
        b.comm_stream.wait_stream(b.default_stream)
        with torch.cuda.stream(b.comm_stream):
            _row_update(b, untouched_rows, zero_grad_rows=True)
            b.side_event = torch.cuda.Event()
            b.side_event.record(b.comm_stream)
        untouched_rows.record_stream(b.comm_stream)


def _cameras_pipelined(b):
    from ...fused import camera_backward, camera_forward_finish, camera_front, camera_loss
    gaussians, bsz, step = b.gaussians, b.bsz, b.step
    sts = _pipeline_streams(gaussians)
    s_front, s_mem, s_raster = sts["mem"][0], sts["mem"][1], sts["raster"][0]
    if getattr(gaussians, "_clmgs_one", None) is None:
        gaussians._clmgs_one = torch.ones((1,), dtype=torch.float32, device=b.params.device)
    for st_ in (s_front, s_mem, s_raster):
        st_.wait_stream(b.default_stream)
    gaussians._clmgs_passes = None
    passes = []
    dp_recv0 = [None]

    def backward(k):
        with _lib.host_region("camera_backward"):
            camera_backward(gaussians, passes[k], b.grad_buf, b.small_gk, stats_delta=b.stats_d,
                            sh_stamp=b.ft_stamp, cur_step=step, release=True)
        if b.dp_split and k == bsz - 2:
            ev = torch.cuda.Event()
            ev.record(s_mem)
            b.dp_comm.wait_event(ev)
            with torch.cuda.stream(b.dp_comm), dp.phase("D0"):
                dp_recv0[0] = dp.border_grads_send([b.grad_buf, b.small_gk], b.ft_stamp, step, b.border, "grads0")

    def catch(k):
        if b.filters[k].numel():
            with torch.cuda.stream(s_front):
                gaussians.catch_up_rows(b.filters[k], to_step=step - 1)
    for k in range(bsz):
        if b.dp_split:
            s_front.wait_event(b.dp_ev_b0 if k == 0 else b.dp_ev_b1)
        if b.split_catch and (k or not b.first_catch_done):
            catch(k)
        if b.split_catch and k == bsz - 1 and getattr(b, "foreign_rows", None) is not None and b.foreign_rows.numel():
            with torch.cuda.stream(s_front):
                gaussians.catch_up_rows(b.foreign_rows, to_step=step - 1)
        with _lib.host_region("camera_front"):
            cur_pass = camera_front(gaussians, b.cameras[k], b.filters[k], b.params.data, 1, b.background,
                                    b.cameras[k].original_image, small_packed=b.small_pk,
                                    streams=(s_front, s_mem, s_raster))
        with _lib.host_region("camera_forward"):
            passes.append(camera_forward_finish(gaussians, cur_pass))
        if k >= 1:
            backward(k - 1)
    backward(bsz - 1)
    if b.dp_split:
        b.default_stream.wait_stream(b.dp_comm)
        gaussians._dp_recv0 = dp_recv0[0]
    for st_ in (s_front, s_mem, s_raster):
        b.default_stream.wait_stream(st_)
    losses = [camera_loss(p_) for p_ in passes]
    gaussians._clmgs_passes = passes
    return losses


def _stage_cameras(b):
    gaussians, args, bsz = b.gaussians, b.args, b.bsz
    b.small_pk = b.small_gk = b.stats_d = None
    if b.use_packed:
        b.small_pk, b.small_gk = gaussians.small_packed(), gaussians.small_grad()
        if (getattr(args, "packed_stats", True) and (not args.disable_auto_densification)
                and utils.get_cur_iter() <= args.densify_until_iter):
            b.stats_d = gaussians.stats_delta()
    else:
        _zero_small_grads(gaussians)
    if b.pipelined:
        return _cameras_pipelined(b)
    losses = []
    if b.fused:
        from ...fused import train_one_camera
        for k in range(bsz):
            losses.append(train_one_camera(
                gaussians, b.cameras[k], b.filters[k], b.params.data, 1, b.grad_buf, b.background,
                b.cameras[k].original_image, small_packed=b.small_pk, small_grad=b.small_gk,
                stats_delta=b.stats_d, sh_stamp=b.ft_stamp, cur_step=b.step))
        return losses
    for k in range(bsz):
        this_filter = b.filters[k]
        with torch.no_grad():
            shs = torch.empty((this_filter.shape[0], 48), device=b.params.device)
            send_shs2gpu_stream(shs, b.params.data, this_filter)
            shs_grad = torch.zeros_like(shs)
        loss = _render_and_backward(gaussians, b.scene, b.cameras[k], b.background, b.pipe_args, this_filter, shs,
                                    shs_grad)
        with torch.no_grad():
            send_shs2cpu_grad_buffer_stream(shs_grad, b.grad_buf, this_filter, True)
        losses.append(loss)
    return losses


def _stage_exchange_tail(b):
    if not dp.active():
        return
    gaussians, N, step = b.gaussians, b.N, b.step
    grad_buf, small_gk, ft_stamp, border = b.grad_buf, b.small_gk, b.ft_stamp, b.border
    if border is not None and b.locality_sparse:
        small_grads = [gaussians._xyz.grad, gaussians._opacity.grad, gaussians._scaling.grad, gaussians._rotation.grad]
        dp.border_grads_home([grad_buf] + small_grads, None, 0, border)
        own_rows = border.own_rows
        _, got = dp.publish_rows(small_grads, own_rows, N, counts=border.own_counts)
        b.touched = torch.zeros((N,), dtype=torch.bool, device=b.params.device)
        for ids in [own_rows] + got:
            if ids.numel():
                utils.fill_rows(b.touched, ids, True)
        b.touched_rows = own_rows.to(torch.int32)
    elif border is not None:
        if b.dp_split:
            r0 = gaussians._dp_recv0
            gaussians._dp_recv0 = None
            for t_ in (r0[0], r0[1], r0[3]):
                if isinstance(t_, torch.Tensor) and t_.is_cuda:
                    t_.record_stream(b.default_stream)
            with dp.phase("D1"):
                r1 = dp.border_grads_send([grad_buf, small_gk], ft_stamp, step, border, "grads1")
            with dp.phase("D_apply"):
                dp.border_grads_apply([grad_buf, small_gk], ft_stamp, step, border, r0)
                dp.border_grads_apply([grad_buf, small_gk], ft_stamp, step, border, r1)
        else:
            with dp.phase("D"):
                dp.border_grads_home([grad_buf, small_gk], ft_stamp, step, border)
        if not b.small_owner:
            dp.publish_small(small_gk, ft_stamp, step, N, border)
    elif b.owner is not None:
        if b.use_packed:
            dp.allreduce_tables_rows([small_gk], b.touched_rows, N, average=False)
        else:
            dp.allreduce_small_grads([gaussians._xyz.grad, gaussians._opacity.grad,
                                      gaussians._scaling.grad, gaussians._rotation.grad], average=False)
        dp.owner_reduce_rows(grad_buf, b.owner)
    elif b.use_packed:
        with dp.phase("allreduce"):
            dp.allreduce_tables_rows([small_gk, grad_buf], b.touched_rows, N, average=False)
    else:
        dp.allreduce_small_grads([gaussians._xyz.grad, gaussians._opacity.grad,
# ... 178 lines not shown
```

clm_gs_amd/strategies/clm_offload/gaussian_model.py:

```python
import os

import torch
from torch import nn

from ... import utils
from ...host import pinned_empty
from ...optimizer import UnifiedAdam
from ..base_gaussian_model import BaseGaussianModel

_ROW_BUFFERS = ("parameters_buffer", "parameters_grad_buffer", "_exp_avg_buffer", "_exp_avg_sq_buffer")


def _gather_f32(t, idx):
    if not (t.is_cuda and t.dtype == torch.float32 and t.is_contiguous() and idx.dtype == torch.int64):
        return utils.take_rows(t, idx).contiguous()
    from ... import clm_kernels
    m = idx.numel()
    out = torch.empty((m,) + tuple(t.shape[1:]), dtype=t.dtype, device=t.device)
    if m:
        clm_kernels._rows("clmgs_rows_gather", out.view(m, -1), t.view(t.shape[0], -1), None, idx.contiguous(), 0)
    return out


def dp_range(n):
# ... 212 lines not shown
                    tables += [st["exp_avg"], st["exp_avg_sq"]]
        dp.owner_gather_dense(tables, n)
        self.invalidate_small_packed()
        self._small_since, self._small_drift = 0, [0.0, 0.0]

    def small_prepare(self, cameras):
        if self._small_since == 0:
            return
        from ... import dp
        from ...gsplat import visibility_candidates
        if (self._small_since >= int(getattr(self.args, "dp_small_refresh", 8))
                or self._small_drift[1] > float(getattr(self.args, "dp_small_max_log_gain", 0.7))):
            self.small_refresh()
            return
        n = self._xyz.shape[0]
        lo, hi = dp.owner_range(n)
        Ks = torch.stack([c.create_k_on_gpu() if getattr(c, "K", None) is None else c.K for c in cameras])
        viewmats = torch.stack([c.world_view_transform.transpose(0, 1) for c in cameras])
        d_xyz, d_ls = self._small_drift
        import math
        cand = visibility_candidates(self._xyz.data, self._scaling.data, viewmats, Ks, int(utils.get_img_width()),
                                     int(utils.get_img_height()), pos_margin=math.sqrt(3.0) * d_xyz * 1.001 + 1e-12,
                                     scale_gain=math.exp(d_ls) * 1.001, own_lo=lo, own_hi=hi)
        pk = self.small_packed()
        lines = dp.small_fetch(cand, n, pk)
        dp.small_scatter(cand, lines, pk, self._small_params())
        if os.environ.get("CLMGS_DP_DEBUG"):
            self._dbg_cand = cand
            print("DPDEBUG small_prepare rank %d since %d drift %s candidates %d of %d foreign rows" % (
                dp.rank(), self._small_since, self._small_drift, cand.numel(), n - (hi - lo)), flush=True)

    def small_after_step(self):
        import math
        groups = {g["name"]: g for g in self.optimizer.gpu_adam.param_groups}
        b1, b2 = groups["xyz"]["betas"]
        c = (1.0 - b1) / math.sqrt(1.0 - b2) / math.sqrt(1.0 - b1 * b1 / b2) * 1.001
        self._small_drift[0] += c * float(groups["xyz"]["lr"])
        self._small_drift[1] += c * float(groups["scaling"]["lr"])
        self._small_since += 1

    @property
    def small_deferred(self):
        return getattr(self, "_small_def", None) is not None

    def _small_def_tables(self, current_as_of=None):
        sd = self._small_def
        n = self._xyz.shape[0]
        if sd["blk_last"] is None or sd["n"] != n:
            assert self._small_def_clean(), "row count changed with small-attribute steps waiting"
            to = sd["hist"][-1][0] if sd["hist"] else int(current_as_of or 0)
            sd["blk_last"] = torch.full(((n + 255) // 256,), int(to), dtype=torch.int32, device=self._xyz.device)
            sd["n"] = n
        return sd["blk_last"]

    def _small_def_clean(self):
        return not getattr(self, "_small_def_dirty", False)

    def small_defer_record(self, step):
        import math
        sd = self._small_def
        order = self.optimizer.small_groups()
        idx = self.optimizer.advance_steps(order)
        if sd["hist"] and sd["hist"][-1][0] != step - 1:
            self.flush_small()
            sd["hist"] = []
            sd["blk_last"] = None
        self._small_def_tables(current_as_of=step - 1)
        b1, b2 = order[0]["betas"]
        c = (1.0 - b1) / math.sqrt(1.0 - b2) / math.sqrt(1.0 - b1 * b1 / b2) * 1.001
        sd["hist"].append((int(step), [float(g["lr"]) for g in order], int(idx), c * float(order[0]["lr"]),
                           c * float(order[2]["lr"])))
        kmax = self._small_kmax()
        if len(sd["hist"]) > kmax:
            del sd["hist"][:len(sd["hist"]) - kmax]
        self._small_def_dirty = True

    def _small_kmax(self):
        k = getattr(self, "_small_kmax_v", None)
        if k is None:
            from ... import _lib
            k = self._small_kmax_v = int(_lib.lib().clmgs_small_deferred_kmax())
        return k

    def small_catch_up(self, cameras=None):
        import ctypes
        import math
        from ... import _lib
        sd = self._small_def
        if not sd["hist"] or (cameras is None and self._small_def_clean()):
            return None
        order = self.optimizer.small_groups()
        ps, ms, vs = self.optimizer.small_pointers(order)
        hist = sd["hist"][::-1]
        nh = len(hist)
        lr = (ctypes.c_double * (4 * nh))(*[x for h in hist for x in h[1]])
        sidx = (ctypes.c_int32 * nh)(*[h[2] for h in hist])
        pm, sg_, dx, dl = [1e-12], [1.001], 0.0, 0.0
        for h in hist:
            dx += h[3]
            dl += h[4]
            pm.append(math.sqrt(3.0) * dx * 1.001 + 1e-12)
            sg_.append(math.exp(dl) * 1.001)
        pos_margin = (ctypes.c_float * (nh + 1))(*pm)
        scale_gain = (ctypes.c_float * (nh + 1))(*sg_)
        pk, gk, blk = self.small_packed(), self.small_grad(), self._small_def_tables()
        b1, b2 = order[0]["betas"]
        C, vm, Ks, flags = 0, None, None, None
        if cameras is not None:
            C = len(cameras)
            flags = sd.get("blk_flag")
            if flags is None or flags.shape[0] != blk.shape[0]:
                flags = sd["blk_flag"] = torch.empty((blk.shape[0],), dtype=torch.uint8, device=blk.device)
            Ks = torch.stack([c.create_k_on_gpu() if getattr(c, "K", None) is None else c.K for c in cameras]).contiguous()
            vm = torch.stack([c.world_view_transform.transpose(0, 1) for c in cameras]).contiguous()
        _lib.check(_lib.lib().clmgs_adam_small_deferred(
            _lib.stream(), int(self._xyz.shape[0]), ps, ms, vs, _lib.dptr(pk), _lib.dptr(gk),
            _lib.dptr(self._row_g_step, torch.int32), _lib.dptr(blk, torch.int32), int(hist[0][0]), nh, lr, sidx,
            pos_margin, scale_gain, float(b1), float(b2), float(order[0]["eps"]), 1.0 / float(self.args.bsz), C,
            _lib.dptr(vm, None, True), _lib.dptr(Ks, None, True), int(utils.get_img_width()), int(utils.get_img_height()),
            0.3, 0.01, 1e10, 0 if cameras is not None else 1, _lib.dptr(flags, torch.uint8, True)))
        if cameras is None:
            self._small_def_dirty = False
        return flags

    def flush_small(self):
        if self.small_deferred:
            self.small_catch_up(None)

    @property
    def lazy_rows(self):
        return getattr(self, "_row_last_step", None) is not None

    @property
    def first_touch_grads(self):
        from ... import dp
        a = self.args
        dp_ok = (not dp.active()) or bool(getattr(a, "dp_locality", False))
        return bool(self.lazy_rows and getattr(a, "fused_front_end", True) and getattr(a, "first_touch_grads", True)
                    and dp_ok and not self.deferred_host_rows and not getattr(a, "mcmc", False))

    @property
    def moments_sharded(self):
        return bool(getattr(self, "_mom_sharded", False))

    @staticmethod
    def _moment_capacity(cap):
        from ... import dp
        return -(-int(cap) // dp.world_size()) + 1

    def catch_up_rows(self, rows=None, to_step=None):
        if not self.lazy_rows:
            return
        if self.moments_sharded and rows is None:
            lo = self._mom_lo
            hi = lo + self.optimizer.cpu_adam.state[self._parameters]["exp_avg"].shape[0]
            if hi <= lo:
                return
            rows = torch.arange(lo, hi, dtype=torch.int32, device=self._xyz.device)
        from ...clm_kernels import adam_catch_up
        opt = self.optimizer.cpu_adam
        g = opt.param_groups[0]
        p = self._parameters
        st = opt.state[p]
        to_step = opt.global_step if to_step is None else to_step
        if to_step <= 0:
            return
        col_lr = opt._col_lr(p.device)
        from ... import dp
        adam_catch_up(p.data, st["exp_avg"], st["exp_avg_sq"], self._row_last_step, rows, col_lr,
                      g["betas"][0], g["betas"][1], g["eps"], to_step, g["bias_correction"],
                      g=self.parameters_grad_buffer[:p.shape[0]], g_step=self._row_g_step,
                      grad_scale=1.0 / (self.args.bsz * dp.world_size()), keep_grad=self.first_touch_grads,
                      moment_row0=self._mom_lo if self.moments_sharded else 0)

    def flush_lazy_rows(self, exchange=True):
        if self.deferred_host_rows:
            self.host_rows_prepare(None, None)
            return
        self.flush_small()
        from ... import dp
        if (not self.lazy_rows) and dp.active() and getattr(self.args, "dp_locality", False) \
                and getattr(self.args, "sparse_adam", False):
            if getattr(self, "_owner_dirty", True) and exchange:
                self._owner_dirty = False
                n = self._parameters.shape[0]
                st = self.optimizer.cpu_adam.state[self._parameters]
                dp.owner_gather_dense([self._parameters.data, st["exp_avg"], st["exp_avg_sq"]], n)
            return
        if self.lazy_rows and dp.active() and (getattr(self.args, "dp_owner_computes", False)
                                               or getattr(self.args, "dp_locality", False)):
            if not getattr(self, "_owner_dirty", True):
                return
            n = self._parameters.shape[0]
            lo, hi = dp.owner_range(n)
            if hi > lo:
                self.catch_up_rows(torch.arange(lo, hi, dtype=torch.int32, device=self._xyz.device))
            if not exchange:
                return
            self._owner_dirty = False
            st = self.optimizer.cpu_adam.state[self._parameters]
            tables = [self._parameters.data]
            if not self.moments_sharded:
                tables += [st["exp_avg"], st["exp_avg_sq"]]
            if not self.first_touch_grads:
                tables.append(self.parameters_grad_buffer[:n])
            dp.owner_gather_dense(tables, n)
# ... 422 lines not shown
```

clm_gs_amd/utils.py:

```python
import io
import time
from types import SimpleNamespace

import numpy as np
import torch

ARGS = None
LOG_FILE = None
CUR_ITER = 0
IMG_W = 0
IMG_H = 0
TIMERS = None
DENSIFY_ITER = 0


def default_args(**over):
    a = SimpleNamespace(
        no_offload=False, naive_offload=False, clm_offload=False, prealloc_capacity=-1,
        comm_stream_priority=-1, grid_size_H=32, grid_size_D=128,
        reorder_by_min_sparsity_at_end=True, sparse_adam=False, gpu=0, packed=False,
        sh_degree=3, radius_clip=0.0, white_background=False,
        iterations=30_000, position_lr_init=0.00016, position_lr_final=0.0000016,
        position_lr_delay_mult=0.01, position_lr_max_steps=30_000, feature_lr=0.0025,
        opacity_lr=0.05, scaling_lr=0.005, lr_scale_loss=1.0, lr_scale_pos_and_scale=1.0,
        rotation_lr=0.001, percent_dense=0.01, lambda_dssim=0.2, densification_interval=100,
        opacity_reset_interval=3000, densify_from_iter=500, densify_until_iter=15_000,
        densify_grad_threshold=0.0002, disable_auto_densification=False, min_opacity=0.005,
        absgrad=False,
        rasterize_mode="classic",
        exposure=False, exposure_lr_init=0.01, exposure_lr_final=0.001,
        depths="", depth_l1_weight_init=1.0, depth_l1_weight_final=0.01,
        mcmc=False, mcmc_cap_max=1_000_000, mcmc_noise_lr=5e5, mcmc_refine_start_iter=500, mcmc_refine_stop_iter=25_000,
        mcmc_refine_every=100, mcmc_min_opacity=0.005, mcmc_opacity_reg=0.01, mcmc_scale_reg=0.01,
        lr_scale_mode="sqrt", bsz=1, exact_filter=True, log_cpu_adam_trailing_overhead=False,
        stop_update_param=False, drop_initial_3dgs_p=0.0,
        debug_skip_optimizer=False,
        sh_residency="hbm",
        fused_front_end=True,
        overlap_cameras=True,
        packed_small=True, packed_stats=True, exact_tile_cull=True,
        sync_each_batch=False,
        dp_overlap=True,
        dp_shard_moments=True,
        dp_small_owner=True,
        dp_small_refresh=8,
        dp_small_max_log_gain=0.7,
        binning="tile",
        deferred_small_adam=True,
        allocator_reservoir=True,
        split_catch_up=True,
        early_first_catch_up=True,
        warm_structural_ops=True,
        defer_loss_log=True,
        spatial_row_order=True,
        first_touch_grads=True,
        host_staging="window",
        placement_candidates=1,
        sh_hbm_budget_gb=0.0,
        host_speculative_prefetch=True,
        device_side_counts=True,
        isect_capacity_margin=1.25,
        isect_capacity_floor=4096,
        reference_camera_order=False,
        dp_locality=False,
        dp_owner_computes=False,
        lazy_dense_adam=True,
    )
    for k, v in over.items():
        setattr(a, k, v)
    return a


RASTERIZE_MODES = ("classic", "antialiased")


def antialiased():
    mode = getattr(ARGS, "rasterize_mode", "classic")
    if mode not in RASTERIZE_MODES:
        raise ValueError(f"rasterize_mode must be one of {RASTERIZE_MODES}, got {mode!r}")
    return mode == "antialiased"


def depth_l1_weight(iteration=None):
    a = get_args()
    it = get_cur_iter() if iteration is None else iteration
    return float(get_expon_lr_func(float(getattr(a, "depth_l1_weight_init", 1.0)),
                                   float(getattr(a, "depth_l1_weight_final", 0.01)),
                                   max_steps=int(getattr(a, "iterations", 30_000)))(int(it)))


class _NullLog(io.StringIO):
    def write(self, s):
        return len(s)


class Timers:
    def __init__(self):
        self.t = {}
        self.acc = {}

    def start(self, k):
        self.t[k] = time.perf_counter()

    def stop(self, k):
        if k in self.t:
            self.acc[k] = self.acc.get(k, 0.0) + time.perf_counter() - self.t.pop(k)


def set_args(a):
    global ARGS
    ARGS = a


def get_args():
    global ARGS
    if ARGS is None:
        ARGS = default_args()
    return ARGS


def set_log_file(f):
    global LOG_FILE
    LOG_FILE = f


def get_log_file():
    global LOG_FILE
    if LOG_FILE is None:
        LOG_FILE = _NullLog()
    return LOG_FILE

# ... 154 lines not shown
```

include/clmgs.h:

```cpp
#ifndef CLMGS_H
#define CLMGS_H
#include <stddef.h>
#include <stdint.h>

#ifdef __cplusplus
extern "C" {
#endif

#define CLMGS_EINVAL 10001
#define CLMGS_ENOMEM 10002

int clmgs_version(void);
const char* clmgs_last_error(void);

int clmgs_projection_fwd(void* stream, int C, int N, const float* means, const float* quats,
                         const float* scales, const float* viewmats, const float* Ks, int width,
                         int height, float eps2d, float near_plane, float far_plane,
                         float radius_clip, int32_t* radii, float* means2d, float* depths,
                         float* conics);
int clmgs_visibility_raw(void* stream, int C, int N, const float* means, const float* quats_raw,
                         const float* log_scales, const float* viewmats, const float* Ks, int width,
                         int height, float eps2d, float near_plane, float far_plane,
                         float radius_clip, int32_t* radii);

size_t clmgs_visibility_select_temp_bytes(int C, int N);
int clmgs_visibility_select_count(void* stream, int C, int N, const float* means,
                                  const float* quats_raw, const float* log_scales,
                                  const float* viewmats, const float* Ks, int width, int height,
                                  float eps2d, float near_plane, float far_plane, float radius_clip,
                                  void* temp, size_t temp_bytes, int64_t* cum_totals);
int clmgs_visibility_select_count_blocks(void* stream, int C, int N, const float* means, const float* quats_raw,
                                         const float* log_scales, const float* viewmats, const float* Ks, int width,
                                         int height, float eps2d, float near_plane, float far_plane, float radius_clip,
                                         void* temp, size_t temp_bytes, int64_t* cum_totals,
                                         const uint8_t* block_flags);
int clmgs_visibility_select_emit(void* stream, int C, int N, const void* temp, int64_t* out);
int clmgs_projection_bwd(void* stream, int C, int N, const float* means, const float* quats,
                         const float* scales, const float* viewmats, const float* Ks, int width,
                         int height, float eps2d, const int32_t* radii, const float* v_means2d,
                         const float* v_depths, const float* v_conics, float* v_means,
                         float* v_quats, float* v_scales);

int clmgs_projection_aa_fwd(void* stream, int C, int N, const float* means, const float* quats,
                            const float* scales, const float* viewmats, const float* Ks, int width,
                            int height, float eps2d, float near_plane, float far_plane,
                            float radius_clip, int32_t* radii, float* means2d, float* depths,
                            float* conics, float* compensations);
int clmgs_projection_aa_bwd(void* stream, int C, int N, const float* means, const float* quats,
                            const float* scales, const float* viewmats, const float* Ks, int width,
                            int height, float eps2d, const int32_t* radii, const float* v_means2d,
                            const float* v_depths, const float* v_conics, const float* v_compensations,
                            float* v_means, float* v_quats, float* v_scales);

int clmgs_sh_fwd(void* stream, int n, int degree, const float* dirs, const float* coeffs,
                 const uint8_t* masks, float* colors);
int clmgs_sh_bwd(void* stream, int n, int degree, const float* dirs, const float* coeffs,
                 const uint8_t* masks, const float* v_colors, float* v_coeffs, int accumulate,
                 float* v_dirs);

size_t clmgs_isect_count_temp_bytes(int CN);
int clmgs_isect_count(void* stream, int C, int N, const float* means2d, const int32_t* radii,
                      int tile_size, int tile_width, int tile_height, int32_t* tiles_per_gauss,
                      int64_t* cum, void* temp, size_t temp_bytes);
size_t clmgs_isect_sort_temp_bytes(int64_t n_isects);
int clmgs_isect_emit_sort(void* stream, int C, int N, int64_t n_isects, const float* means2d,
                          const int32_t* radii, const float* depths, const int64_t* cum,
                          int tile_size, int tile_width, int tile_height, int64_t* isect_ids,
                          int32_t* flatten_ids, void* temp, size_t temp_bytes);
int clmgs_isect_offsets(void* stream, int64_t n_isects, const int64_t* isect_ids, int C,
                        int tile_width, int tile_height, int32_t* offsets);

size_t clmgs_isect2_order_temp_bytes(int V);
int clmgs_isect2_order_count(void* stream, int V, const float* means2d, const int32_t* radii,
                             const float* depths, int tile_size, int tile_width, int tile_height,
                             const void* packed, int32_t* order, int64_t* cum, uint64_t* boxes,
                             int64_t* totals, void* temp, size_t temp_bytes, int64_t* row_cum);
size_t clmgs_isect2_sort_temp_bytes(int64_t n_isects);
int clmgs_isect2_emit_sort(void* stream, int V, int64_t n_isects, const float* depths,
                           const int32_t* order, const int64_t* cum, const uint64_t* boxes,
                           int tile_width, int tile_height, int32_t* flatten_ids, int32_t* offsets,
                           int64_t* isect_ids, int32_t* emit_slot, void* temp, size_t temp_bytes,
                           const int64_t* row_cum);

size_t clmgs_rasterize_pack_bytes(int C, int N);
int clmgs_rasterize_fwd(void* stream, int C, int N, int64_t n_isects, const float* means2d,
                        const float* conics, const float* colors, const float* opacities,
                        const float* backgrounds, int width, int height, int tile_size,
                        int tile_width, int tile_height, const int32_t* offsets,
                        const int32_t* flatten_ids, void* packed, float* render_colors,
                        float* render_alphas, int32_t* last_ids);
size_t clmgs_rasterize_partials_bytes(int64_t n_isects);
int clmgs_rasterize_bwd(void* stream, int C, int N, int64_t n_isects, const void* packed,
                        const float* backgrounds, int width, int height, int tile_size,
                        int tile_width, int tile_height, const int32_t* offsets,
                        const int32_t* flatten_ids, const float* render_alphas,
                        const int32_t* last_ids, const float* v_render_colors,
                        const float* v_render_alphas, void* packed_grad, float* v_means2d,
                        float* v_conics, float* v_colors, float* v_opacities,
                        const int32_t* emit_slot, const int64_t* row_cum, void* partials);

int clmgs_rasterize4_fwd(void* stream, int C, int N, int64_t n_isects, const float* means2d,
                         const float* conics, const float* colors, const float* opacities,
                         const float* backgrounds, int width, int height, int tile_size,
                         int tile_width, int tile_height, const int32_t* offsets,
                         const int32_t* flatten_ids, void* packed, float* render_colors,
                         float* render_alphas, int32_t* last_ids);
int clmgs_rasterize4_bwd(void* stream, int C, int N, int64_t n_isects, const void* packed,
                         const float* backgrounds, int width, int height, int tile_size,
                         int tile_width, int tile_height, const int32_t* offsets,
                         const int32_t* flatten_ids, const float* render_alphas,
                         const int32_t* last_ids, const float* v_render_colors,
                         const float* v_render_alphas, void* packed_grad, float* v_means2d,
                         float* v_conics, float* v_colors, float* v_opacities,
                         const int32_t* emit_slot, const int64_t* row_cum, void* partials);
int clmgs_rasterize4_slot_bwd(void* stream, int C, int N, int64_t n_isects, const void* packed,
                              const float* backgrounds, int width, int height, int tile_size,
                              int tile_width, int tile_height, const int32_t* offsets,
                              const int32_t* flatten_ids, const float* render_alphas,
                              const int32_t* last_ids, const float* v_render_colors,
// ... 180 lines not shown
                      int grid_blocks);
int clmgs_rows_scatter_add(void* stream, float* dst, const float* src, const void* dst_idx,
                           const void* src_idx, int idx_is_64, int64_t n_rows, int cols,
                           int grid_blocks);

int clmgs_scatter_to_bit(void* stream, void* bitmap, int elem_bytes, const int64_t* filter,
                         int64_t n, int bit);
int clmgs_extract_ffs(void* stream, const void* bitmap, int elem_bytes, int64_t N, uint8_t* ffs);
int clmgs_pair_overlap_count(void* stream, const void* bitmap, int elem_bytes, int64_t N,
                             int bsz, int32_t* cnt);
int clmgs_set_signal(void* stream, int32_t* signal_pinned, int idx, int32_t value);

int clmgs_adam_rows(void* stream, float* p, float* g, float* m, float* v, const void* rows,
                    int idx_is_64, const uint8_t* mask, int64_t n_rows, int cols,
                    const float* col_lr, double beta1, double beta2, double eps, int step,
                    int bias_correction, float grad_scale, int zero_grad);
int clmgs_pack_small(void* stream, int64_t n, const float* xyz, const float* opacity,
                     const float* scaling, const float* rotation, void* packed_p);
int clmgs_adam_small_packed(void* stream, int64_t n, float* const* params, float* const* exp_avg,
                            float* const* exp_avg_sq, const double* lr4, void* packed_p,
                            void* packed_g, double beta1, double beta2, double eps, int step,
                            int bias_correction, float grad_scale, const int32_t* g_stamp, int cur_step);
int clmgs_adam_catch_up(void* stream, float* p, float* m, float* v, const int32_t* last_step,
                        const void* rows, int idx_is_64, int64_t n_rows, int cols,
                        const float* col_lr, double beta1, double beta2, double eps, int to_step,
                        int bias_correction, int max_replay, float* g, const int32_t* g_step,
                        float grad_scale, int keep_grad);
int clmgs_host_adam_rows(float* p, float* g, float* m, float* v, const int32_t* rows,
                         int64_t n_rows, int cols, const float* col_lr, double beta1,
                         double beta2, double eps, int step, int bias_correction, float grad_scale,
                         int zero_grad, const volatile int32_t* signal, int n_threads);

int clmgs_host_pool_start(int n_threads);
int clmgs_host_usable_cpus(void);
int clmgs_memcpy_async(void* stream, void* dst, const void* src, size_t bytes, int kind);
int clmgs_host_rows_prepare(float* p, const float* g, float* m, float* v, int32_t* last_step,
                            int32_t* g_step, const int32_t* rows, int64_t n_rows, int cols,
                            const float* col_lr, double beta1, double beta2, double eps, int to_step,
                            int next_g_step, int bias_correction, float grad_scale, int max_replay,
                            float* stage, int sparse);

int clmgs_densify_stats(void* stream, int64_t n, const int64_t* filter, const float* v_means2d,
                        const int32_t* radii, int only_visible, float half_w, float half_h,
                        float* max_radii2D,
                        float* xyz_gradient_accum, float* denom);

size_t clmgs_morton_order_temp_bytes(int64_t n);
int clmgs_morton_order(void* stream, int64_t n, const float* xyz, const double* lo_hi, int64_t* order, void* temp,
                       size_t temp_bytes);

int clmgs_tsp_tour(int n, const int64_t* dist, int32_t* tour);

int clmgs_knn3_mean_dist2(void* stream, int n, const float* pts_sorted, const int32_t* cell_start,
                          float ox, float oy, float oz, float h, int gx, int gy, int gz,
                          int max_ring, float* mean_d2_sorted);

size_t clmgs_host_groups_temp_bytes(int64_t n);
int clmgs_host_groups(void* stream, int64_t n, const int64_t* touched, const void* bitmap, int elem_bytes, int bsz,
                      const uint8_t* staged, int slot0, int32_t* late_sorted, int32_t* rows_by_last, int32_t* slot_of,
                      int64_t* counts, void* temp, size_t temp_bytes);

int clmgs_publish_pack(void* stream, float* msg, const float* table, const int64_t* own_rows, const int32_t* stamp,
                       int step, int64_t lo, int64_t n_rows, int64_t chunk, int cols);

int clmgs_visibility_candidates(void* stream, int C, int N, int own_lo, int own_hi, const float* means,
                                const float* log_scales, const float* viewmats, const float* Ks, int width,
                                int height, float eps2d, float near_plane, float far_plane, float pos_margin,
                                float scale_gain, uint8_t* mask);
int clmgs_small_rows_scatter(void* stream, int64_t n_rows, const int64_t* rows, const void* lines, float* xyz,
                             float* opacity, float* scaling, float* rotation, void* packed_p);
int clmgs_adam_small_packed_range(void* stream, int64_t n, int64_t row_begin, int64_t row_end, float* const* params,
                                  float* const* exp_avg, float* const* exp_avg_sq, const double* lr4, void* packed_p,
                                  void* packed_g, double beta1, double beta2, double eps, int step,
                                  int bias_correction, float grad_scale, const int32_t* g_stamp, int cur_step);

int clmgs_small_deferred_kmax(void);
int clmgs_adam_small_deferred(void* stream, int64_t n, float* const* params, float* const* exp_avg,
                              float* const* exp_avg_sq, void* packed_p, const void* packed_g, const int32_t* g_stamp,
                              int32_t* blk_last, int to_step, int n_hist, const double* lr4_hist,
                              const int32_t* step_index, const float* pos_margin, const float* scale_gain, double beta1,
                              double beta2, double eps, float grad_scale, int C, const float* viewmats, const float* Ks,
                              int width, int height, float eps2d, float near_plane, float far_plane, int flush_all,
                              uint8_t* blk_flag );

int clmgs_device_errors(uint32_t* bits, int reset);

void* clmgs_pinned_alloc(size_t bytes);
int clmgs_pinned_free(void* p);

#ifdef __cplusplus
}
#endif
#endif
```

profiles/make_pmc_json.py:

```python
import ast
import json
import re
import sys

GROUPS = {
    "clmgs_rasterize_bwd": ["rasterize_bwd_kernel"],
    "clmgs_rasterize_fwd": ["rasterize_fwd_kernel"],
    "clmgs_l1_ssim_loss_fwd": ["loss_fwd_kernel"],
    "clmgs_l1_ssim_loss_bwd": ["loss_bwd_kernel"],
    "clmgs_preprocess_fwd": ["preprocess_fwd_kernel"],
    "clmgs_preprocess_bwd": ["preprocess_bwd_kernel"],
    "clmgs_adam_rows": ["adam_rows_kernel"],
    "clmgs_adam_catch_up": ["adam_catch_up"],
    "clmgs_adam_small_deferred": ["adam_small_deferred_kernel"],
    "clmgs_isect3_front": ["isect3_rows_kernel", "isect3_rows_finish_kernel"],
    "clmgs_isect3_bin": ["isect3_tile_scan_kernel", "isect3_scatter_kernel", "isect3_sort_"],
}


MEDIAN_KERNELS = ("adam_catch_up",)


def _lines(path):
    rows = []
    for line in open(path):
        m = re.match(r"(.*?) (\{.*?\}) launches (\d+)(?: median (\{.*\}))?", line.strip())
        if m:
            mean = ast.literal_eval(m.group(2))
            med = ast.literal_eval(m.group(4)) if m.group(4) else mean
            rows.append((m.group(1), mean, med, int(m.group(3))))
    for x in MEDIAN_KERNELS:
        fam = [r for r in rows if x in r[0]]
        if len(fam) > 1:
            keep = max(fam, key=lambda r: r[3])
            rows = [r for r in rows if r not in fam or r is keep]
    for name, mean, med, _n in rows:
        yield name, (med if any(x in name for x in MEDIAN_KERNELS) else mean)


def read(path, counter):
    return {k: d[counter] * 1024.0 for k, d in _lines(path) if counter in d}


def read_raw(path, counter):
    return {k: d[counter] for k, d in _lines(path) if counter in d}


f, w = read(sys.argv[1], "FETCH_SIZE"), read(sys.argv[2], "WRITE_SIZE")
sq = read_raw(sys.argv[3], "SQ_INSTS_VALU") if len(sys.argv) > 3 else {}
label = sys.argv[4] if len(sys.argv) > 4 else "this round's build"
algo = {}
if len(sys.argv) > 5:
    for line in open(sys.argv[5]):
        if line.startswith("{"):
            j = json.loads(line)
            for name, k in (j.get("kernels") or {}).items():
                if "algo_GBps" in k:
                    algo[name] = k["algo_GBps"] * 1e9 * k["avg_ms"] * 1e-3
            rf = j.get("roofline") or {}
            if rf.get("kernel") and rf.get("algo_bytes_per_launch"):
                algo[rf["kernel"]] = rf["algo_bytes_per_launch"]
res = {"_note": "rocprofv3 --pmc FETCH_SIZE / WRITE_SIZE (separate passes, --kernel-trace only), KB per launch "
                "averaged over the launches of `bench.py --steps 1 --warmup 1`; bytes = KB*1024, summed over "
                "the device kernels of one C-ABI call. MI355X guide: FETCH_SIZE reports 1/2 of wide coalesced "
                "reads on gfx950 (x2 applied in fetch_bytes_x2); other widths and WRITE_SIZE uncalibrated. "
                "traffic = fetch_bytes_x2 + write_bytes.",
       "rubble28m": {}}
for entry, kernels in GROUPS.items():
    fr = sum(v for k, v in f.items() if any(x in k for x in kernels) and "unsigned long" not in k)
    wr = sum(v for k, v in w.items() if any(x in k for x in kernels) and "unsigned long" not in k)
    if fr + wr == 0:
        continue
    res["rubble28m"][entry] = {"fetch_bytes_raw": fr, "fetch_bytes_x2": 2 * fr, "write_bytes": wr,
                               "traffic": 2 * fr + wr}
    if entry in algo:
        res["rubble28m"][entry]["algo_bytes"] = round(algo[entry], 1)
        res["rubble28m"][entry]["traffic_over_algo"] = round((2 * fr + wr) / algo[entry], 3)
    if any(x in k for k in list(f) + list(w) for x in kernels if x in MEDIAN_KERNELS):
        res["rubble28m"][entry]["launch"] = "median launch of the per-camera passes (split_catch_up: four per batch; the whole-table flush excluded)"
    vi = sum(v for k, v in sq.items() if any(x in k for x in kernels) and "unsigned long" not in k)
    if vi:
        res["rubble28m"][entry]["valu_insts"] = vi
res["_source"] = "rocprofv3 --pmc passes of " + label + " (profiles/collect_r06.sh)"
json.dump(res, open(__file__.replace("make_pmc_json.py", "pmc_traffic.json"), "w"), indent=1)
print(json.dumps(res["rubble28m"], indent=1))
```

profiles/timeline.py:

```python
import sqlite3
import sys

db = sys.argv[1]
arg = sys.argv[2] if len(sys.argv) > 2 else "150"
c = sqlite3.connect(db)
rows = list(c.execute("select name, start, end, stream_id from kernels order by start"))
if arg.startswith("step"):
    marks = [r[1] for r in rows if "visibility_bits" in r[0]]
    k = int(arg[4:] or 2)
    t0, t_end = marks[-k - 1], marks[-k]
    rows = [r for r in rows if t0 <= r[1] < t_end]
    print(f"{len(rows)} kernels in batch -{k} of the trace ({(t_end - t0) / 1e6:.2f} ms between two visibility_bits launches)")
else:
    win_ms = float(arg)
    t_end = max(r[2] for r in rows)
    t0 = t_end - win_ms * 1e6
    rows = [r for r in rows if r[1] >= t0]
    print(f"{len(rows)} kernels in the last {win_ms} ms")
iv = sorted((r[1], r[2]) for r in rows)
busy, cur_s, cur_e = 0, iv[0][0], iv[0][1]
gaps = []
for s, e in iv[1:]:
    if s > cur_e:
        busy += cur_e - cur_s
        gaps.append((s - cur_e, cur_e))
        cur_s, cur_e = s, e
    else:
        cur_e = max(cur_e, e)
busy += cur_e - cur_s
span = (t_end - t0) if arg.startswith("step") else iv[-1][1] - iv[0][0]
ksum = sum(e - s for s, e in iv)
print(f"span {span/1e6:.2f} ms, GPU busy (union) {busy/1e6:.2f} ms = {100*busy/span:.1f}%, "
      f"sum of kernel durations {ksum/1e6:.2f} ms = {ksum/max(busy,1):.2f}x the busy time (concurrency)")
tot = {}
for n, s, e, st in rows:
    k = n.split("(")[0][-60:]
    a = tot.setdefault(k, [0, 0.0])
    a[0] += 1
    a[1] += (e - s) / 1e6
for k, (n, ms) in sorted(tot.items(), key=lambda kv: -kv[1][1])[:30]:
    print(f"{ms:8.2f} ms n={n:4d}  {k}")
print("largest idle gaps:")
for g, at in sorted(gaps, reverse=True)[:14]:
    prev = [r for r in rows if r[2] <= at + 1][-1][0].split("(")[0][-50:]
    nxt = [r for r in rows if r[1] >= at + g - 1][0][0].split("(")[0][-50:]
    print(f"  {g/1e6:6.3f} ms at t-{(t_end-at)/1e6:7.2f} ms  after {prev}  before {nxt}")
```

profiles/timeline_host.py:

```python
import sqlite3
import sys

c = sqlite3.connect(sys.argv[1])
arg = sys.argv[2] if len(sys.argv) > 2 else None
win = float(arg) * 1e6 if arg and not arg.startswith("batches") else None
names = [r[0] for r in c.execute("select name from sqlite_master where type in ('table','view')")]
kern = list(c.execute("select name, start, end from kernels order by start"))
mc_view = next((n for n in names if n.lower() in ("memory_copies", "memory_copy")), None) or \
    next((n for n in names if "memory_cop" in n.lower() and "rocpd_" not in n.lower()), None) or \
    next((n for n in names if "memory_cop" in n.lower()), None)
copies = []
if mc_view:
    cols = [r[1] for r in c.execute(f"pragma table_info('{mc_view}')")]
    sc, ec = ("start" if "start" in cols else "start_timestamp"), ("end" if "end" in cols else "end_timestamp")
    size_c = next((x for x in cols if x in ("size", "bytes", "size_bytes")), None)
    name_c = next((x for x in cols if x in ("name", "kind", "direction")), None)
    q = f"select {sc}, {ec}, {size_c or 0}, {name_c or 0} from {mc_view} order by {sc}"
    copies = [(s, e, b, str(n)) for s, e, b, n in c.execute(q)]
t_end = max([k[2] for k in kern] + [x[1] for x in copies])
t0 = t_end - win if win else min(k[1] for k in kern)
if arg and arg.startswith("batches"):
    marks = [k[1] for k in kern if "visibility_bits" in k[0]]
    nb = int(arg[7:] or 2)
    t0, t_end = marks[-nb - 1], marks[-1]
kern = [k for k in kern if t0 <= k[1] < t_end]
copies = [x for x in copies if t0 <= x[0] < t_end]
scatter = [(s, e) for n, s, e in kern if "rows_move_f4_kernel" in n]
render = sorted((s, e) for n, s, e in kern if "rows_move_f4_kernel" not in n)


def union(iv):
    out = []
    for s, e in sorted(iv):
        if out and s <= out[-1][1]:
            out[-1][1] = max(out[-1][1], e)
        else:
            out.append([s, e])
    return out


def overlap(a, b):
    i = j = 0
    tot = 0
    while i < len(a) and j < len(b):
        lo, hi = max(a[i][0], b[j][0]), min(a[i][1], b[j][1])
        if hi > lo:
            tot += hi - lo
        if a[i][1] < b[j][1]:
            i += 1
        else:
            j += 1
    return tot


ru = union(render)
span = t_end - t0
print(f"window {span / 1e6:.1f} ms; render kernels busy {sum(e - s for s, e in ru) / 1e6:.1f} ms")
print(f"copy view: {mc_view}; {len(copies)} SDMA copies, {len(scatter)} zero-copy scatter launches")
by = {}
for s, e, b, n in copies:
    a = by.setdefault(n, [0, 0, 0.0])
    a[0] += 1; a[1] += int(b or 0); a[2] += (e - s)
for n, (k, b, t) in by.items():
    print(f"  {n}: n={k} bytes={b / 1e9:.3f} GB busy={t / 1e6:.1f} ms -> {b / max(t, 1):.1f} GB/s while active")
for label, iv in (("SDMA copies", [(s, e) for s, e, _, _ in copies]), ("zero-copy gradient scatter", scatter),
                  ("all link traffic", [(s, e) for s, e, _, _ in copies] + scatter)):
    u = union(iv)
    tot = sum(e - s for s, e in u)
    if tot:
        print(f"{label}: active {tot / 1e6:.1f} ms ({100 * tot / span:.0f}% of the window), "
              f"{100 * overlap(u, ru) / tot:.0f}% of it under render kernels")
```

profiles/timeline_streams.py:

```python
import sqlite3
import sys

db = sys.argv[1]
arg = sys.argv[2] if len(sys.argv) > 2 else "31"
c = sqlite3.connect(db)
rows = list(c.execute("select name, start, end, queue_id, grid_x, workgroup_x, lds_size from kernels order by start"))
if arg.startswith("step"):
    marks = [r[1] for r in rows if "visibility_bits" in r[0]]
    k = int(arg[4:] or 2)
    t0, t_end = marks[-k - 1], marks[-k]
    rows = [r for r in rows if t0 <= r[1] < t_end]
else:
    t_end = max(r[2] for r in rows)
    t0 = t_end - float(arg) * 1e6
    rows = [r for r in rows if r[1] >= t0]
KEYS = ("rasterize_bwd", "rasterize_fwd", "partials_sum", "preprocess_bwd", "preprocess_fwd", "loss_bwd",
        "loss_fwd", "adam_rows", "adam_small", "catch_up", "radix_scan_rows", "radix_scatter",
        "radix_onesweep", "radix_hist_all", "radix_hist", "radix_scan_digits", "isect2_keys", "isect2_count",
        "isect2_emit", "isect2_offsets", "scan_i64_blocks", "scan_i64_totals", "scan_i64_add",
        "visibility_bits", "visibility_emit", "copyBuffer", "fillBuffer", "index_put", "direct_copy")


def short(n):
    n = n.split("(")[0]
    for k in KEYS:
        if k in n:
            return k
    return n[-28:]


queues = sorted(set(r[3] for r in rows))
print("queues:", queues)
for n, s, e, q, gx, wx, lds in rows:
    print(f"{(s - t0) / 1e6:8.3f} {(e - s) / 1e3:8.1f}us  q{queues.index(q)}  {short(n):18s} grid {gx // max(wx, 1)}x{wx} lds {lds}")
print()
raster_q = None
for q in queues:
    mine = [r for r in rows if r[3] == q]
    busy = sum(r[2] - r[1] for r in mine)
    n_r = sum(1 for r in mine if "rasterize" in r[0])
    print(f"q{queues.index(q)}: {len(mine)} kernels, busy {busy / 1e6:.2f} ms, tile kernels {n_r}")
    if n_r and (raster_q is None or n_r > raster_q[1]):
        raster_q = (q, n_r)
if raster_q:
    q = raster_q[0]
    mine = [r for r in rows if r[3] == q]
    print(f"\nidle gaps of q{queues.index(q)} (tile kernels) > 50 us and the other queues' kernels inside them:")
    for a, b in zip(mine[:-1], mine[1:]):
        gap = b[1] - a[2]
        if gap > 50e3:
            inside = [r for r in rows if r[3] != q and r[2] > a[2] and r[1] < b[1]]
            desc = ", ".join(f"{short(r[0])}:{(min(r[2], b[1]) - max(r[1], a[2])) / 1e3:.0f}" for r in inside)
            print(f"  {gap / 1e3:7.0f} us after {short(a[0])} at {(a[2] - t0) / 1e6:.2f} ms: {desc}")
```

Before: 195.2.

## Fuse deferred small-attribute Adam catch-up with per-batch visibility selection

Adds a templated SELECT variant of the deferred small-Adam kernel that computes per-camera visibility bits and counts for each block right after updating its parameters, while they are still in LDS. The separate visibility_bits pass over means, scales and quaternions is dropped when the fused batch head is enabled. The shared visibility-classification code is factored into helpers so both kernels use it. The fused kernel needs more LDS and registers, which may lower occupancy, and it puts the visibility work on the catch-up kernel's critical path. A u32 union emit entry point is also added.

```diff
diff --git a/clm_gs_amd/_lib.py b/clm_gs_amd/_lib.py
--- a/clm_gs_amd/_lib.py
+++ b/clm_gs_amd/_lib.py
@@ -18,6 +18,7 @@
     "clmgs_visibility_select_count": (_i, [_vp, _i, _i, _vp, _vp, _vp, _vp, _vp, _i, _i, _f, _f, _f, _f, _vp, _sz, _vp]),
     "clmgs_visibility_select_count_blocks": (_i, [_vp, _i, _i, _vp, _vp, _vp, _vp, _vp, _i, _i, _f, _f, _f, _f, _vp, _sz, _vp, _vp]),
     "clmgs_visibility_select_emit": (_i, [_vp, _i, _i, _vp, _vp]),
+    "clmgs_visibility_select_emit_u32": (_i, [_vp, _i, _i, _vp, _vp, _vp]),
     "clmgs_visibility_raw": (_i, [_vp, _i, _i, _vp, _vp, _vp, _vp, _vp, _i, _i, _f, _f, _f, _f, _vp]),
     "clmgs_projection_bwd": (_i, [_vp, _i, _i, _vp, _vp, _vp, _vp, _vp, _i, _i, _f, _vp, _vp, _vp, _vp, _vp, _vp, _vp]),
     "clmgs_sh_fwd": (_i, [_vp, _i, _i, _vp, _vp, _vp, _vp]),
@@ -106,6 +107,8 @@
     "clmgs_small_deferred_kmax": (_i, []),
     "clmgs_adam_small_deferred": (_i, [_vp, _i64, _vp, _vp, _vp, _vp, _vp, _vp, _vp, _i, _i, _vp, _vp, _vp, _vp, _d, _d, _d,
                                        _f, _i, _vp, _vp, _i, _i, _f, _f, _f, _i, _vp]),
+    "clmgs_adam_small_deferred_select": (_i, [_vp, _i64, _vp, _vp, _vp, _vp, _vp, _vp, _vp, _i, _i, _vp, _vp, _vp, _vp, _d,
+                                              _d, _d, _f, _i, _vp, _vp, _i, _i, _f, _f, _f, _vp, _vp, _f, _vp, _sz, _vp]),
     "clmgs_device_errors": (_i, [_vp, _i]),
     "clmgs_pinned_alloc": (_vp, [_sz]),
     "clmgs_pinned_free": (_i, [_vp]),
diff --git a/clm_gs_amd/csrc/clm_ops.hip b/clm_gs_amd/csrc/clm_ops.hip
--- a/clm_gs_amd/csrc/clm_ops.hip
+++ b/clm_gs_amd/csrc/clm_ops.hip
@@ -532,17 +532,34 @@
   int to_step;
 };
 
+struct SmallSelect {
+  float radius_clip;
+  int W64;
+  unsigned long long* bits;
+  int64_t* counts;
+};
+
+template <bool SELECT>
 __global__ void __launch_bounds__(SA_ROWS)
 adam_small_deferred_kernel(int64_t n, SmallAdam t, float4* __restrict__ packed_p, const float4* __restrict__ packed_g,
                            const int32_t* __restrict__ g_stamp, int32_t* __restrict__ blk_last, SmallDeferred d,
                            float beta1, float beta2, float ob1, float ob2, float eps, float grad_scale, int C,
                            const float* __restrict__ viewmats, const float* __restrict__ Ks, float W, float H, float eps2d,
                            float near_plane, float far_plane, int flush_all, uint8_t* __restrict__ blk_flag, int n_hist,
-                           uint32_t* __restrict__ dev_err) {
+                           uint32_t* __restrict__ dev_err, SmallSelect sel) {
   __shared__ __attribute__((aligned(16))) float sg[SA_ROWS * 12];
   __shared__ __attribute__((aligned(16))) float sp[SA_ROWS * 12];
   __shared__ int gstep_s[SA_ROWS];
   __shared__ float cam_s[VB_MAX_CAMS][VB_CAM_F];
+  VisBlockLds vl = {};
+  if constexpr (SELECT) {
+    __shared__ unsigned short vcand[SA_ROWS * VB_CH];
+    __shared__ int vn_cand;
+    __shared__ unsigned long long vwb[VB_CH][4];
+    __shared__ unsigned long long vanyw[4];
+    static_assert(SA_ROWS == 256 && sizeof(sg) >= SA_ROWS * 10 * sizeof(float));
+    vl = {reinterpret_cast<float (*)[10]>(sg), vcand, &vn_cand, vwb, vanyw};
+  }
   const int tid = threadIdx.x;
   if (!flush_all) {
     for (int c = tid; c < C; c += SA_ROWS) vis_store_cam(cam_s[c], viewmats + 16 * c, Ks + 9 * c, W, H);
@@ -561,13 +578,19 @@
     const int64_t row0 = blk * SA_ROWS;
     const int rows = (int)min((int64_t)SA_ROWS, n - row0);
     __syncthreads();
+    bool sel_any = false;
     if (!flush_all) {
       const int kk = min(max(k, 0), SD_KMAX);
       bool cand = false;
+      float sm[3] = {0.f, 0.f, 0.f}, sl[3] = {0.f, 0.f, 0.f};
       if (tid < rows) {
         const float* x = t.p[0] + 3 * (row0 + tid);
         const float* ls = t.p[2] + 3 * (row0 + tid);
         const float m[3] = {x[0], x[1], x[2]};
+        if constexpr (SELECT) {
+          sm[0] = m[0]; sm[1] = m[1]; sm[2] = m[2];
+          sl[0] = ls[0]; sl[1] = ls[1]; sl[2] = ls[2];
+        }
         const float sgn = __expf(fmaxf(ls[0], fmaxf(ls[1], ls[2]))) * d.scale_gain[kk];
         const float smax2g = sgn * sgn;
         cand = !(smax2g < 1e30f);
@@ -576,6 +599,17 @@
       }
       const bool any = __syncthreads_or(cand);
       if (blk_flag && tid == 0) blk_flag[blk] = any ? 1 : 0;
+      if constexpr (SELECT) {
+        sel_any = any;
+        if (!any) {
+          vis_block_zero(C, (int)blk, sel.W64, sel.bits, sel.counts);
+        } else if (k <= 0) {
+          float4 q4 = make_float4(0.f, 0.f, 0.f, 0.f);
+          if (tid < rows) q4 = *reinterpret_cast<const float4*>(t.p[3] + 4 * (row0 + tid));
+          vis_block_bits(vl, cam_s, C, (int)blk, sel.W64, tid < rows, sm, q4, __expf(sl[0]), __expf(sl[1]), __expf(sl[2]),
+                         viewmats, Ks, W, H, eps2d, near_plane, far_plane, sel.radius_clip, sel.bits, sel.counts);
+        }
+      }
       if (k <= 0 || (!any && k < SD_KMAX)) continue;
     }
     if (tid < rows) {
@@ -601,6 +635,17 @@
     });
     for (int i = tid; i < rows * 3; i += SA_ROWS) packed_p[row0 * 3 + i] = reinterpret_cast<const float4*>(sp)[i];
     if (tid == 0) blk_last[blk] = d.to_step;
+    if constexpr (SELECT) {
+      if (sel_any) {
+        const bool in = tid < rows;
+        const float* r = sp + (in ? tid : 0) * 12;
+        const float m[3] = {r[0], r[1], r[2]};
+        const float4 q4 = make_float4(r[7], r[8], r[9], r[10]);
+        const float s0 = __expf(r[4]), s1 = __expf(r[5]), s2 = __expf(r[6]);
+        vis_block_bits(vl, cam_s, C, (int)blk, sel.W64, in, m, q4, s0, s1, s2, viewmats, Ks, W, H, eps2d, near_plane,
+                       far_plane, sel.radius_clip, sel.bits, sel.counts);
+      }
+    }
   }
 }
 
@@ -991,6 +1036,49 @@
 
 extern "C" int clmgs_small_deferred_kmax(void) { return SD_KMAX; }
 
+static int adam_small_deferred_impl(void* stream, int64_t n, float* const* params, float* const* exp_avg,
+                                    float* const* exp_avg_sq, void* packed_p, const void* packed_g,
+                                    const int32_t* g_stamp, int32_t* blk_last, int to_step, int n_hist,
+                                    const double* lr4_hist, const int32_t* step_index, const float* pos_margin,
+                                    const float* scale_gain, double beta1, double beta2, double eps,
+                                    float grad_scale, int C, const float* viewmats, const float* Ks, int width,
+                                    int height, float eps2d, float near_plane, float far_plane, int flush_all,
+                                    uint8_t* blk_flag, const SmallSelect* sel) {
+  CLMGS_CHECK_ARG(packed_p && packed_g && g_stamp && blk_last && lr4_hist && step_index && pos_margin && scale_gain &&
+                  (((uintptr_t)packed_p | (uintptr_t)packed_g) & 15) == 0);
+  CLMGS_CHECK_ARG(flush_all || (C >= 1 && C <= VB_MAX_CAMS && viewmats && Ks && width > 0 && height > 0));
+  SmallAdam t;
+  CLMGS_CHECK_ARG(small_adam_fill(&t, params, exp_avg, exp_avg_sq, nullptr));
+  SmallDeferred d;
+  for (int j = 0; j < SD_KMAX; ++j) {
+    const int jj = j < n_hist ? j : n_hist - 1;
+    for (int i = 0; i < 4; ++i) d.lr[j][i] = (float)lr4_hist[4 * jj + i];
+    CLMGS_CHECK_ARG(step_index[jj] >= 1);
+    adam_bias_host(beta1, beta2, step_index[jj], 1, &d.inv_bc1[j], &d.inv_sqrt_bc2[j]);
+  }
+  for (int k = 0; k <= SD_KMAX; ++k) {
+    const int kk = k <= n_hist ? k : n_hist;
+    d.pos_margin[k] = pos_margin[kk];
+    d.scale_gain[k] = scale_gain[kk];
+  }
+  d.to_step = to_step;
+  const float ob1 = (float)(1.0 - beta1), ob2 = (float)(1.0 - beta2);
+  const dim3 grid(min(ceil_div(n, SA_ROWS), 256 * 16));
+  if (sel)
+    hipLaunchKernelGGL(adam_small_deferred_kernel<true>, grid, dim3(SA_ROWS), 0,
+                       (hipStream_t)stream, n, t, (float4*)packed_p, (const float4*)packed_g, g_stamp, blk_last, d,
+                       (float)beta1, (float)beta2, ob1, ob2, (float)eps, grad_scale, C, viewmats, Ks, (float)width,
+                       (float)height, eps2d, near_plane, far_plane, flush_all, blk_flag, n_hist, device_error_word(), *sel);
+  else
+    hipLaunchKernelGGL(adam_small_deferred_kernel<false>, grid, dim3(SA_ROWS), 0,
+                       (hipStream_t)stream, n, t, (float4*)packed_p, (const float4*)packed_g, g_stamp, blk_last, d,
+                       (float)beta1, (float)beta2, ob1, ob2, (float)eps, grad_scale, C, viewmats, Ks, (float)width,
+                       (float)height, eps2d, near_plane, far_plane, flush_all, blk_flag, n_hist, device_error_word(),
+                       SmallSelect{});
+  CLMGS_LAUNCH_CHECK();
+  return 0;
+}
+
 extern "C" int clmgs_adam_small_deferred(void* stream, int64_t n, float* const* params, float* const* exp_avg,
                                          float* const* exp_avg_sq, void* packed_p, const void* packed_g,
                                          const int32_t* g_stamp, int32_t* blk_last, int to_step, int n_hist,
@@ -1006,31 +1094,43 @@
     if (blk_flag) CLMGS_HIP(hipMemsetAsync(blk_flag, 1, (size_t)((n + SA_ROWS - 1) / SA_ROWS), (hipStream_t)stream));
     return 0;
   }
-  CLMGS_CHECK_ARG(packed_p && packed_g && g_stamp && blk_last && lr4_hist && step_index && pos_margin && scale_gain &&
-                  (((uintptr_t)packed_p | (uintptr_t)packed_g) & 15) == 0);
-  CLMGS_CHECK_ARG(flush_all || (C >= 1 && C <= VB_MAX_CAMS && viewmats && Ks && width > 0 && height > 0));
-  SmallAdam t;
-  CLMGS_CHECK_ARG(small_adam_fill(&t, params, exp_avg, exp_avg_sq, nullptr));
-  SmallDeferred d;
-  for (int j = 0; j < SD_KMAX; ++j) {
-    const int jj = j < n_hist ? j : n_hist - 1;
-    for (int i = 0; i < 4; ++i) d.lr[j][i] = (float)lr4_hist[4 * jj + i];
-    CLMGS_CHECK_ARG(step_index[jj] >= 1);
-    adam_bias_host(beta1, beta2, step_index[jj], 1, &d.inv_bc1[j], &d.inv_sqrt_bc2[j]);
-  }
-  for (int k = 0; k <= SD_KMAX; ++k) {
-    const int kk = k <= n_hist ? k : n_hist;
-    d.pos_margin[k] = pos_margin[kk];
-    d.scale_gain[k] = scale_gain[kk];
-  }
-  d.to_step = to_step;
-  const float ob1 = (float)(1.0 - beta1), ob2 = (float)(1.0 - beta2);
-  hipLaunchKernelGGL(adam_small_deferred_kernel, dim3(min(ceil_div(n, SA_ROWS), 256 * 16)), dim3(SA_ROWS), 0,
-                     (hipStream_t)stream, n, t, (float4*)packed_p, (const float4*)packed_g, g_stamp, blk_last, d,
-                     (float)beta1, (float)beta2, ob1, ob2, (float)eps, grad_scale, C, viewmats, Ks, (float)width,
-                     (float)height, eps2d, near_plane, far_plane, flush_all, blk_flag, n_hist, device_error_word());
-  CLMGS_LAUNCH_CHECK();
-  return 0;
+  return adam_small_deferred_impl(stream, n, params, exp_avg, exp_avg_sq, packed_p, packed_g, g_stamp, blk_last, to_step,
+                                  n_hist, lr4_hist, step_index, pos_margin, scale_gain, beta1, beta2, eps, grad_scale, C,
+                                  viewmats, Ks, width, height, eps2d, near_plane, far_plane, flush_all, blk_flag, nullptr);
+}
+
+extern "C" int clmgs_adam_small_deferred_select(void* stream, int64_t n, float* const* params, float* const* exp_avg,
+                                                float* const* exp_avg_sq, void* packed_p, const void* packed_g,
+                                                const int32_t* g_stamp, int32_t* blk_last, int to_step, int n_hist,
+                                                const double* lr4_hist, const int32_t* step_index,
+                                                const float* pos_margin, const float* scale_gain, double beta1,
+                                                double beta2, double eps, float grad_scale, int C, const float* viewmats,
+                                                const float* Ks, int width, int height, float eps2d, float near_plane,
+                                                float far_plane, uint8_t* blk_flag, const float* quats_raw,
+                                                float radius_clip, void* temp, size_t temp_bytes, int64_t* cum_totals) {
+  CLMGS_CHECK_ARG(n >= 1 && n <= INT32_MAX && to_step >= 0 && n_hist >= 0 && n_hist <= SD_KMAX);
+  CLMGS_CHECK_ARG(C >= 1 && C <= VB_MAX_CAMS && viewmats && Ks && width > 0 && height > 0);
+  CLMGS_CHECK_ARG(blk_flag && temp && cum_totals && params && params[0] && params[2] && params[3]);
+  CLMGS_CHECK_ARG(quats_raw == params[3]);
+  CLMGS_CHECK_ARG(temp_bytes >= clmgs_visibility_select_temp_bytes(C, (int)n));
+  if (n_hist == 0) {
+    const int rc = clmgs_adam_small_deferred(stream, n, params, exp_avg, exp_avg_sq, packed_p, packed_g, g_stamp, blk_last,
+                                             to_step, n_hist, lr4_hist, step_index, pos_margin, scale_gain, beta1, beta2,
+                                             eps, grad_scale, C, viewmats, Ks, width, height, eps2d, near_plane, far_plane,
+                                             0, blk_flag);
+    if (rc) return rc;
+    return clmgs_visibility_select_count_blocks(stream, C, (int)n, params[0], quats_raw, params[2], viewmats, Ks, width,
+                                                height, eps2d, near_plane, far_plane, radius_clip, temp, temp_bytes,
+                                                cum_totals, blk_flag);
+  }
+  const VisSelectTemp vt = vis_select_temp(C, (int)n, temp);
+  const SmallSelect sel = {radius_clip, vt.W64, vt.bits, vt.counts};
+  const int rc = adam_small_deferred_impl(stream, n, params, exp_avg, exp_avg_sq, packed_p, packed_g, g_stamp, blk_last,
+                                          to_step, n_hist, lr4_hist, step_index, pos_margin, scale_gain, beta1, beta2, eps,
+                                          grad_scale, C, viewmats, Ks, width, height, eps2d, near_plane, far_plane, 0,
+                                          blk_flag, &sel);
+  if (rc) return rc;
+  return vis_select_scan_totals((hipStream_t)stream, C, vt, cum_totals);
 }
 
 extern "C" int clmgs_device_errors(uint32_t* out, int reset) {
diff --git a/clm_gs_amd/csrc/isect.hip b/clm_gs_amd/csrc/isect.hip
--- a/clm_gs_amd/csrc/isect.hip
+++ b/clm_gs_amd/csrc/isect.hip
@@ -537,24 +537,6 @@
 
 namespace clmgs {
 
-constexpr int VB_CH = 4;
-
-__device__ __forceinline__ int vis_classify(const Cam& c, float kc, const float m[3], float smax2,
-                                            float W, float H, float eps2d, float near_m, float far_m,
-                                            float near_p, float far_p, bool accept_ok) {
-  const float x = c.R[0] * m[0] + c.R[1] * m[1] + c.R[2] * m[2] + c.t[0];
-  const float y = c.R[3] * m[0] + c.R[4] * m[1] + c.R[5] * m[2] + c.t[1];
-  const float z = c.R[6] * m[0] + c.R[7] * m[1] + c.R[8] * m[2] + c.t[2];
-  if (z < near_m || z > far_m) return 0;
-  const float rz = __builtin_amdgcn_rcpf(z);
-  const float mx = c.fx * x * rz + c.cx, my = c.fy * y * rz + c.cy;
-  const float B = smax2 * rz * rz * kc + eps2d;
-  if (accept_ok && z > near_p && z < far_p && B < 400.f && mx >= 1.f && mx <= W - 1.f && my >= 1.f &&
-      my <= H - 1.f)
-    return 1;
-  const float Rb = 3.03f * __builtin_amdgcn_sqrtf(2.f * B + 0.1f) + 2.f;
-  return (mx + Rb <= 0.f || mx - Rb >= W || my + Rb <= 0.f || my - Rb >= H) ? 0 : 2;
-}
 
 __global__ void __launch_bounds__(256)
 visibility_bits_kernel(int C, int N, int W64, const float* __restrict__ means,
@@ -569,22 +551,9 @@
   __shared__ int n_cand;
   __shared__ unsigned long long wb[VB_CH][4];
   __shared__ unsigned long long anyw[4];
-  const int tid = threadIdx.x, lane = tid & 63;
-  const unsigned long long lt = (1ull << lane) - 1ull;
-  const float near_m = near_plane - (fabsf(near_plane) * 1e-5f + 1e-6f);
-  const float far_m = far_plane + fabsf(far_plane) * 1e-5f;
-  const float near_p = near_plane + (fabsf(near_plane) * 1e-5f + 1e-6f);
-  const float far_p = far_plane - fabsf(far_plane) * 1e-5f;
-  const bool accept_ok = radius_clip < 1.5f && eps2d >= 0.3f;
-  const int wid = tid >> 6;
-  for (int c = tid; c < C; c += 256) {
-    const Cam cam = load_cam(viewmats + 16 * c, Ks + 9 * c);
-    float* f = cam_s[c];
-    for (int i = 0; i < 9; ++i) f[i] = cam.R[i];
-    f[9] = cam.t[0]; f[10] = cam.t[1]; f[11] = cam.t[2];
-    f[12] = cam.fx; f[13] = cam.fy; f[14] = cam.cx; f[15] = cam.cy;
-    f[16] = vis_cam_kc(cam, W, H);
-  }
+  const VisBlockLds lds = {row_s, cand, &n_cand, wb, anyw};
+  const int tid = threadIdx.x;
+  for (int c = tid; c < C; c += 256) vis_store_cam(cam_s[c], viewmats + 16 * c, Ks + 9 * c, W, H);
   const int n_rb = (W64 + 3) / 4;
   float nm0 = 0.f, nm1 = 0.f, nm2 = 0.f, nl0 = 0.f, nl1 = 0.f, nl2 = 0.f;
   float4 nq = make_float4(0.f, 0.f, 0.f, 0.f);
@@ -605,73 +574,11 @@
     const float s0 = __expf(nl0), s1 = __expf(nl1), s2 = __expf(nl2);
     fetch(rb + gridDim.x);
     if (blk_flag && !blk_flag[rb]) {
-      if (tid < (C + 1) * 4) {
-        const int c = tid >> 2, w = rb * 4 + (tid & 3);
-        if (w < W64) { bits[(size_t)c * W64 + w] = 0ull; counts[(size_t)c * W64 + w] = 0; }
-      }
-      for (int q = tid + 256; q < (C + 1) * 4; q += 256) {
-        const int c = q >> 2, w = rb * 4 + (q & 3);
-        if (w < W64) { bits[(size_t)c * W64 + w] = 0ull; counts[(size_t)c * W64 + w] = 0; }
-      }
+      vis_block_zero(C, rb, W64, bits, counts);
       continue;
     }
-    const float smax = fmaxf(s0, fmaxf(s1, s2));
-    const float smax2 = smax * smax;
-    const float qn2 = q4.x * q4.x + q4.y * q4.y + q4.z * q4.z + q4.w * q4.w;
-    const bool row_ok = accept_ok && qn2 >= 1e-20f && qn2 <= 1e20f && (s0 + s1 + s2) < 1e30f;
-    lds_barrier();
-    {
-      float* r = row_s[tid];
-      r[0] = m[0]; r[1] = m[1]; r[2] = m[2]; r[3] = q4.x; r[4] = q4.y; r[5] = q4.z; r[6] = q4.w;
-      r[7] = s0; r[8] = s1; r[9] = s2;
-    }
-    if (tid < 4) anyw[tid] = 0ull;
-    for (int c0 = 0; c0 < C; c0 += VB_CH) {
-      const int cn = min(VB_CH, C - c0);
-      if (tid < VB_CH * 4) wb[tid >> 2][tid & 3] = 0ull;
-      if (tid == 0) n_cand = 0;
-      lds_barrier();
-      for (int cc = 0; cc < cn; ++cc) {
-        const Cam cam = load_cam(viewmats + 16 * (c0 + cc), Ks + 9 * (c0 + cc));
-        const int cls = in ? vis_classify(cam, cam_s[c0 + cc][16], m, smax2, W, H, eps2d, near_m, far_m,
-                                          near_p, far_p, row_ok) : 0;
-        const unsigned long long acc = __ballot(cls == 1);
-        if (lane == 0 && acc) atomicOr(&wb[cc][wid], acc);
-        const bool pass = cls == 2;
-        const unsigned long long b = __ballot(pass);
-        int base = 0;
-        if (lane == 0 && b) base = atomicAdd(&n_cand, __popcll(b));
-        base = __builtin_amdgcn_readfirstlane(base);
-        if (pass) cand[base + __popcll(b & lt)] = (unsigned short)(tid | (cc << 8));
-      }
-      lds_barrier();
-      const int nc = n_cand;
-      for (int k = tid; k < nc; k += 256) {
-        const int e = cand[k], r = e & 255, cc = e >> 8;
-        const Cam cam = lds_cam(cam_s[c0 + cc]);
-        const float* rr = row_s[r];
-        const float mm[3] = {rr[0], rr[1], rr[2]};
-        const float qq[4] = {rr[3], rr[4], rr[5], rr[6]};
-        const float ss[3] = {rr[7], rr[8], rr[9]};
-        const Proj p = project_fwd(cam, mm, qq, ss, W, H, eps2d, near_plane, far_plane, radius_clip);
-        if (p.radius > 0) atomicOr(&wb[cc][r >> 6], 1ull << (r & 63));
-      }
-      lds_barrier();
-      if (tid < cn * 4) {
-        const int cc = tid >> 2, j = tid & 3, w = rb * 4 + j;
-        if (w < W64) {
-          const unsigned long long b = wb[cc][j];
-          bits[(size_t)(c0 + cc) * W64 + w] = b;
-          counts[(size_t)(c0 + cc) * W64 + w] = __popcll(b);
-          if (b) atomicOr(&anyw[j], b);
-        }
-      }
-    }
-    lds_barrier();
-    if (tid < 4 && rb * 4 + tid < W64) {
-      bits[(size_t)C * W64 + rb * 4 + tid] = anyw[tid];
-      counts[(size_t)C * W64 + rb * 4 + tid] = __popcll(anyw[tid]);
-    }
+    vis_block_bits(lds, cam_s, C, rb, W64, in, m, q4, s0, s1, s2, viewmats, Ks, W, H, eps2d, near_plane, far_plane,
+                   radius_clip, bits, counts);
   }
 }
 
@@ -709,10 +616,12 @@
   }
 }
 
+template <bool U32>
 __global__ void __launch_bounds__(256)
 visibility_emit_kernel(int C, int N, int W64, const unsigned long long* __restrict__ bits,
-                       const int64_t* __restrict__ scan, int64_t* __restrict__ out) {
+                       const int64_t* __restrict__ scan, int64_t* __restrict__ out, int32_t* __restrict__ union32) {
   const int64_t total = (int64_t)(C + 1) * W64 * 64;
+  const int64_t word_u = (int64_t)C * W64;
   for (int64_t t = blockIdx.x * (int64_t)blockDim.x + threadIdx.x; t < total;
        t += (int64_t)gridDim.x * blockDim.x) {
     const int64_t word = t >> 6;
@@ -723,8 +632,34 @@
       const int64_t pos = end - __popcll(b) + __popcll(b & ((1ull << bit) - 1ull));
       const int w = (int)(word % W64);
       out[pos] = (int64_t)w * 64 + bit;
-    }
-  }
+      if (U32 && word >= word_u) union32[pos - scan[word_u - 1]] = w * 64 + bit;
+    }
+  }
+}
+
+__global__ void __launch_bounds__(128)
+visibility_totals_kernel(int C, int W64, const int64_t* __restrict__ scan, int64_t* __restrict__ cum_totals) {
+  const int r = threadIdx.x;
+  if (r <= C) cum_totals[r] = scan[(size_t)(r + 1) * W64 - 1];
+}
+
+VisSelectTemp vis_select_temp(int C, int N, void* temp) {
+  VisSelectTemp t;
+  t.W64 = (N + 63) / 64;
+  const size_t words = (size_t)(C + 1) * t.W64;
+  char* base = (char*)temp;
+  t.bits = (unsigned long long*)base; base += align_up(words * 8, 256);
+  t.counts = (int64_t*)base; base += align_up(words * 8, 256);
+  t.scratch = (int64_t*)base;
+  return t;
+}
+
+int vis_select_scan_totals(hipStream_t s, int C, const VisSelectTemp& t, int64_t* cum_totals) {
+  const int rc = inclusive_scan_i64(s, (int64_t)(C + 1) * t.W64, t.counts, t.scratch);
+  if (rc) return rc;
+  hipLaunchKernelGGL(visibility_totals_kernel, dim3(1), dim3(128), 0, s, C, t.W64, t.counts, cum_totals);
+  CLMGS_LAUNCH_CHECK();
+  return 0;
 }
 
 }
@@ -762,36 +697,38 @@
   CLMGS_CHECK_ARG(means && quats_raw && log_scales && viewmats && Ks && temp && cum_totals);
   CLMGS_CHECK_ARG(temp_bytes >= clmgs_visibility_select_temp_bytes(C, N));
   hipStream_t s = (hipStream_t)stream;
-  const int W64 = (N + 63) / 64;
-  const size_t words = (size_t)(C + 1) * W64;
-  char* base = (char*)temp;
-  unsigned long long* bits = (unsigned long long*)base; base += align_up(words * 8, 256);
-  int64_t* counts = (int64_t*)base; base += align_up(words * 8, 256);
-  int64_t* scratch = (int64_t*)base;
-  hipLaunchKernelGGL(visibility_bits_kernel, dim3(min(ceil_div((int64_t)W64 * 64, 256), 256 * 8)),
-                     dim3(256), 0, s, C, N, W64, means, quats_raw, log_scales, viewmats, Ks,
-                     (float)width, (float)height, eps2d, near_plane, far_plane, radius_clip, bits, counts, block_flags);
-  CLMGS_LAUNCH_CHECK();
-  const int rc = inclusive_scan_i64(s, (int64_t)words, counts, scratch);
-  if (rc) return rc;
-  for (int r = 0; r <= C; ++r)
-    CLMGS_HIP(hipMemcpyAsync(cum_totals + r, counts + (size_t)(r + 1) * W64 - 1, sizeof(int64_t),
-                             hipMemcpyDeviceToDevice, s));
+  const VisSelectTemp t = vis_select_temp(C, N, temp);
+  hipLaunchKernelGGL(visibility_bits_kernel, dim3(min(ceil_div((int64_t)t.W64 * 64, 256), 256 * 8)),
+                     dim3(256), 0, s, C, N, t.W64, means, quats_raw, log_scales, viewmats, Ks,
+                     (float)width, (float)height, eps2d, near_plane, far_plane, radius_clip, t.bits, t.counts, block_flags);
+  CLMGS_LAUNCH_CHECK();
+  return vis_select_scan_totals(s, C, t, cum_totals);
+}
+
+static int visibility_emit_impl(void* stream, int C, int N, const void* temp, int64_t* out, int32_t* union32) {
+  CLMGS_CHECK_ARG(C >= 1 && N >= 1 && temp && out);
+  const VisSelectTemp t = vis_select_temp(C, N, const_cast<void*>(temp));
+  const size_t words = (size_t)(C + 1) * t.W64;
+  const dim3 grid(min(ceil_div((int64_t)words * 64, 256), 256 * 32));
+  if (union32)
+    hipLaunchKernelGGL(visibility_emit_kernel<true>, grid, dim3(256), 0, (hipStream_t)stream, C, N, t.W64, t.bits, t.counts,
+                       out, union32);
+  else
+    hipLaunchKernelGGL(visibility_emit_kernel<false>, grid, dim3(256), 0, (hipStream_t)stream, C, N, t.W64, t.bits,
+                       t.counts, out, union32);
+  CLMGS_LAUNCH_CHECK();
   return 0;
 }
 
 extern "C" int clmgs_visibility_select_emit(void* stream, int C, int N, const void* temp,
                                             int64_t* out) {
-  CLMGS_CHECK_ARG(C >= 1 && N >= 1 && temp && out);
-  const int W64 = (N + 63) / 64;
-  const size_t words = (size_t)(C + 1) * W64;
-  const char* base = (const char*)temp;
-  const unsigned long long* bits = (const unsigned long long*)base; base += align_up(words * 8, 256);
-  const int64_t* scan = (const int64_t*)base;
-  hipLaunchKernelGGL(visibility_emit_kernel, dim3(min(ceil_div((int64_t)words * 64, 256), 256 * 32)),
-                     dim3(256), 0, (hipStream_t)stream, C, N, W64, bits, scan, out);
-  CLMGS_LAUNCH_CHECK();
-  return 0;
+  return visibility_emit_impl(stream, C, N, temp, out, nullptr);
+}
+
+extern "C" int clmgs_visibility_select_emit_u32(void* stream, int C, int N, const void* temp, int64_t* out,
+                                                int32_t* union32) {
+  CLMGS_CHECK_ARG(union32);
+  return visibility_emit_impl(stream, C, N, temp, out, union32);
 }
 
 
diff --git a/clm_gs_amd/csrc/vis_math.h b/clm_gs_amd/csrc/vis_math.h
--- a/clm_gs_amd/csrc/vis_math.h
+++ b/clm_gs_amd/csrc/vis_math.h
@@ -52,4 +52,130 @@
   f[16] = vis_cam_kc(cam, W, H);
 }
 
+
+constexpr int VB_CH = 4;
+
+__device__ __forceinline__ int vis_classify(const Cam& c, float kc, const float m[3], float smax2,
+                                            float W, float H, float eps2d, float near_m, float far_m,
+                                            float near_p, float far_p, bool accept_ok) {
+  const float x = c.R[0] * m[0] + c.R[1] * m[1] + c.R[2] * m[2] + c.t[0];
+  const float y = c.R[3] * m[0] + c.R[4] * m[1] + c.R[5] * m[2] + c.t[1];
+  const float z = c.R[6] * m[0] + c.R[7] * m[1] + c.R[8] * m[2] + c.t[2];
+  if (z < near_m || z > far_m) return 0;
+  const float rz = __builtin_amdgcn_rcpf(z);
+  const float mx = c.fx * x * rz + c.cx, my = c.fy * y * rz + c.cy;
+  const float B = smax2 * rz * rz * kc + eps2d;
+  if (accept_ok && z > near_p && z < far_p && B < 400.f && mx >= 1.f && mx <= W - 1.f && my >= 1.f &&
+      my <= H - 1.f)
+    return 1;
+  const float Rb = 3.03f * __builtin_amdgcn_sqrtf(2.f * B + 0.1f) + 2.f;
+  return (mx + Rb <= 0.f || mx - Rb >= W || my + Rb <= 0.f || my - Rb >= H) ? 0 : 2;
 }
+
+struct VisBlockLds {
+  float (*row_s)[10];
+  unsigned short* cand;
+  int* n_cand;
+  unsigned long long (*wb)[4];
+  unsigned long long* anyw;
+};
+
+__device__ __forceinline__ void vis_block_zero(int C, int rb, int W64, unsigned long long* __restrict__ bits,
+                                               int64_t* __restrict__ counts) {
+  const int tid = threadIdx.x;
+  if (tid < (C + 1) * 4) {
+    const int c = tid >> 2, w = rb * 4 + (tid & 3);
+    if (w < W64) { bits[(size_t)c * W64 + w] = 0ull; counts[(size_t)c * W64 + w] = 0; }
+  }
+  for (int q = tid + 256; q < (C + 1) * 4; q += 256) {
+    const int c = q >> 2, w = rb * 4 + (q & 3);
+    if (w < W64) { bits[(size_t)c * W64 + w] = 0ull; counts[(size_t)c * W64 + w] = 0; }
+  }
+}
+
+__device__ __forceinline__ void vis_block_bits(const VisBlockLds& L, const float (*cam_s)[VB_CAM_F], int C, int rb, int W64,
+                                               bool in, const float m[3], float4 q4, float s0, float s1, float s2,
+                                               const float* __restrict__ viewmats, const float* __restrict__ Ks, float W,
+                                               float H, float eps2d, float near_plane, float far_plane, float radius_clip,
+                                               unsigned long long* __restrict__ bits, int64_t* __restrict__ counts) {
+  float (*row_s)[10] = L.row_s;
+  unsigned short* cand = L.cand;
+  int& n_cand = *L.n_cand;
+  unsigned long long (*wb)[4] = L.wb;
+  unsigned long long* anyw = L.anyw;
+  const int tid = threadIdx.x, lane = tid & 63, wid = tid >> 6;
+  const unsigned long long lt = (1ull << lane) - 1ull;
+  const float near_m = near_plane - (fabsf(near_plane) * 1e-5f + 1e-6f);
+  const float far_m = far_plane + fabsf(far_plane) * 1e-5f;
+  const float near_p = near_plane + (fabsf(near_plane) * 1e-5f + 1e-6f);
+  const float far_p = far_plane - fabsf(far_plane) * 1e-5f;
+  const bool accept_ok = radius_clip < 1.5f && eps2d >= 0.3f;
+  const float smax = fmaxf(s0, fmaxf(s1, s2));
+  const float smax2 = smax * smax;
+  const float qn2 = q4.x * q4.x + q4.y * q4.y + q4.z * q4.z + q4.w * q4.w;
+  const bool row_ok = accept_ok && qn2 >= 1e-20f && qn2 <= 1e20f && (s0 + s1 + s2) < 1e30f;
+  lds_barrier();
+  {
+    float* r = row_s[tid];
+    r[0] = m[0]; r[1] = m[1]; r[2] = m[2]; r[3] = q4.x; r[4] = q4.y; r[5] = q4.z; r[6] = q4.w;
+    r[7] = s0; r[8] = s1; r[9] = s2;
+  }
+  if (tid < 4) anyw[tid] = 0ull;
+  for (int c0 = 0; c0 < C; c0 += VB_CH) {
+    const int cn = min(VB_CH, C - c0);
+    if (tid < VB_CH * 4) wb[tid >> 2][tid & 3] = 0ull;
+    if (tid == 0) n_cand = 0;
+    lds_barrier();
+    for (int cc = 0; cc < cn; ++cc) {
+      const Cam cam = load_cam(viewmats + 16 * (c0 + cc), Ks + 9 * (c0 + cc));
+      const int cls = in ? vis_classify(cam, cam_s[c0 + cc][16], m, smax2, W, H, eps2d, near_m, far_m,
+                                        near_p, far_p, row_ok) : 0;
+      const unsigned long long acc = __ballot(cls == 1);
+      if (lane == 0 && acc) atomicOr(&wb[cc][wid], acc);
+      const bool pass = cls == 2;
+      const unsigned long long b = __ballot(pass);
+      int base = 0;
+      if (lane == 0 && b) base = atomicAdd(&n_cand, __popcll(b));
+      base = __builtin_amdgcn_readfirstlane(base);
+      if (pass) cand[base + __popcll(b & lt)] = (unsigned short)(tid | (cc << 8));
+    }
+    lds_barrier();
+    const int nc = n_cand;
+    for (int k = tid; k < nc; k += 256) {
+      const int e = cand[k], r = e & 255, cc = e >> 8;
+      const Cam cam = lds_cam(cam_s[c0 + cc]);
+      const float* rr = row_s[r];
+      const float mm[3] = {rr[0], rr[1], rr[2]};
+      const float qq[4] = {rr[3], rr[4], rr[5], rr[6]};
+      const float ss[3] = {rr[7], rr[8], rr[9]};
+      const Proj p = project_fwd(cam, mm, qq, ss, W, H, eps2d, near_plane, far_plane, radius_clip);
+      if (p.radius > 0) atomicOr(&wb[cc][r >> 6], 1ull << (r & 63));
+    }
+    lds_barrier();
+    if (tid < cn * 4) {
+      const int cc = tid >> 2, j = tid & 3, w = rb * 4 + j;
+      if (w < W64) {
+        const unsigned long long b = wb[cc][j];
+        bits[(size_t)(c0 + cc) * W64 + w] = b;
+        counts[(size_t)(c0 + cc) * W64 + w] = __popcll(b);
+        if (b) atomicOr(&anyw[j], b);
+      }
+    }
+  }
+  lds_barrier();
+  if (tid < 4 && rb * 4 + tid < W64) {
+    bits[(size_t)C * W64 + rb * 4 + tid] = anyw[tid];
+    counts[(size_t)C * W64 + rb * 4 + tid] = __popcll(anyw[tid]);
+  }
+}
+
+struct VisSelectTemp {
+  unsigned long long* bits;
+  int64_t* counts;
+  int64_t* scratch;
+  int W64;
+};
+VisSelectTemp vis_select_temp(int C, int N, void* temp);
+int vis_select_scan_totals(hipStream_t s, int C, const VisSelectTemp& t, int64_t* cum_totals);
+
+}
diff --git a/clm_gs_amd/gsplat.py b/clm_gs_amd/gsplat.py
--- a/clm_gs_amd/gsplat.py
+++ b/clm_gs_amd/gsplat.py
@@ -156,7 +156,7 @@
 
 
 def visibility_select(means, quats_raw, log_scales, viewmats, Ks, width, height, eps2d=0.3,
-                      near_plane=0.01, far_plane=1e10, radius_clip=0.0, block_flags=None):
+                      near_plane=0.01, far_plane=1e10, radius_clip=0.0, block_flags=None, count=None, union32=False):
     L = _lib.lib()
     means, quats_raw, log_scales = means.contiguous(), quats_raw.contiguous(), log_scales.contiguous()
     viewmats, Ks = viewmats.contiguous(), Ks.contiguous()
@@ -165,18 +165,27 @@
     tb = L.clmgs_visibility_select_temp_bytes(C, N)
     temp = torch.empty((tb,), dtype=torch.uint8, device=dev)
     cum = torch.empty((C + 1,), dtype=I64, device=dev)
-    check(L.clmgs_visibility_select_count_blocks(
-        stream(), C, N, dptr(means, F32), dptr(quats_raw, F32), dptr(log_scales, F32), dptr(viewmats, F32),
-        dptr(Ks, F32), int(width), int(height), float(eps2d), float(near_plane), float(far_plane),
-        float(radius_clip), dptr(temp), tb, dptr(cum), dptr(block_flags, torch.uint8, True)))
+    if count is not None:
+        count(temp, tb, cum)
+    else:
+        check(L.clmgs_visibility_select_count_blocks(
+            stream(), C, N, dptr(means, F32), dptr(quats_raw, F32), dptr(log_scales, F32), dptr(viewmats, F32),
+            dptr(Ks, F32), int(width), int(height), float(eps2d), float(near_plane), float(far_plane),
+            float(radius_clip), dptr(temp), tb, dptr(cum), dptr(block_flags, torch.uint8, True)))
     _t0 = time.perf_counter()
     ends = cum.tolist()
     _lib.STATS["host_wait_s"] += time.perf_counter() - _t0
     out = torch.empty((max(ends[-1], 1),), dtype=I64, device=dev)
+    starts = [0] + ends[:-1]
+    u32 = torch.empty((max(ends[-1] - starts[-1], 1),), dtype=I32, device=dev) if union32 else None
     if ends[-1] > 0:
-        check(L.clmgs_visibility_select_emit(stream(), C, N, dptr(temp), dptr(out)))
-    starts = [0] + ends[:-1]
+        if union32:
+            check(L.clmgs_visibility_select_emit_u32(stream(), C, N, dptr(temp), dptr(out), dptr(u32, I32)))
+        else:
+            check(L.clmgs_visibility_select_emit(stream(), C, N, dptr(temp), dptr(out)))
     pieces = tuple(out[a:b] for a, b in zip(starts, ends))
+    if union32:
+        return pieces[:C], pieces[C], u32[:ends[-1] - starts[-1]]
     return pieces[:C], pieces[C]
 
 
diff --git a/clm_gs_amd/strategies/clm_offload/engine.py b/clm_gs_amd/strategies/clm_offload/engine.py
--- a/clm_gs_amd/strategies/clm_offload/engine.py
+++ b/clm_gs_amd/strategies/clm_offload/engine.py
@@ -260,12 +260,17 @@
             gaussians.small_prepare(cams)
     b.small_deferred = bool(getattr(gaussians, "small_deferred", False) and b.fused and gaussians.lazy_rows
                             and not args.stop_update_param and getattr(args, "packed_small", True))
-    blk_flags = None
+    blk_flags = sel = None
+    b.touched_rows32 = None
     if b.small_deferred:
-        with torch.no_grad():
-            blk_flags = gaussians.small_catch_up(cams)
+        with torch.no_grad(), _lib.host_region("select_filters"):
+            blk_flags, sel = gaussians.small_catch_up(cams, select={"radius_clip": args.radius_clip, "union32": True})
     with torch.no_grad():
-        if b.fused:
+        if sel is not None:
+            b.filters, b.touched_rows, b.touched_rows32 = sel
+            assert all(f.numel() > 0 for f in b.filters), (
+                "every camera must see at least one gaussian (base_engine.py:64-67)")
+        elif b.fused:
             with _lib.host_region("select_filters"):
                 b.filters, b.touched_rows = select_filters(cams, gaussians._xyz.detach(), gaussians._scaling.detach(),
                                                            gaussians._rotation.detach(), block_flags=blk_flags)
@@ -316,7 +321,7 @@
         if dp.active() and not b.locality_sparse:
             b.local_touched = b.touched
             b.touched = dp.allreduce_touched(b.touched)
-            b.touched_rows = None
+            b.touched_rows = b.touched_rows32 = None
     b.row_adam = gaussians.optimizer.cpu_adam
     b.params = gaussians._parameters
     b.grad_buf = b.parameters_grad_buffer[:N]
@@ -331,7 +336,10 @@
     b.col_lr = b.row_adam._col_lr(b.params.device)
     if b.touched_rows is None:
         b.touched_rows = torch.nonzero(b.touched).flatten()
-    b.touched_rows = b.touched_rows.to(torch.int32)
+    if getattr(b, "touched_rows32", None) is not None:
+        b.touched_rows = b.touched_rows32
+    else:
+        b.touched_rows = b.touched_rows.to(torch.int32)
     _lib.STATS.setdefault("touched_rows", []).append(int(b.touched_rows.shape[0]))
     b.ft_stamp = gaussians._row_g_step if (b.lazy and b.fused and gaussians.first_touch_grads) else None
 
@@ -471,9 +479,15 @@
     if b.dp_split:
         b.default_stream.wait_stream(b.dp_comm)
         gaussians._dp_recv0 = dp_recv0[0]
+    losses = None
+    if all(p_.ev_loss is not None for p_ in passes):
+        for p_ in passes:
+            b.default_stream.wait_event(p_.ev_loss)
+        losses = [camera_loss(p_) for p_ in passes]
     for st_ in (s_front, s_mem, s_raster):
         b.default_stream.wait_stream(st_)
-    losses = [camera_loss(p_) for p_ in passes]
+    if losses is None:
+        losses = [camera_loss(p_) for p_ in passes]
     gaussians._clmgs_passes = passes
     return losses
 
diff --git a/clm_gs_amd/strategies/clm_offload/gaussian_model.py b/clm_gs_amd/strategies/clm_offload/gaussian_model.py
--- a/clm_gs_amd/strategies/clm_offload/gaussian_model.py
+++ b/clm_gs_amd/strategies/clm_offload/gaussian_model.py
@@ -318,13 +318,20 @@
             k = self._small_kmax_v = int(_lib.lib().clmgs_small_deferred_kmax())
         return k
 
-    def small_catch_up(self, cameras=None):
+    def small_head_fused(self):
+        a = self.args
+        return bool(self.small_deferred and self._small_def["hist"] and not getattr(self, "small_owner", False)
+                    and getattr(a, "fused_front_end", True) and getattr(a, "fused_batch_head", True)
+                    and not getattr(a, "reference_camera_order", False))
+
+    def small_catch_up(self, cameras=None, select=None):
         import ctypes
         import math
         from ... import _lib
         sd = self._small_def
+        fused = cameras is not None and select is not None and self.small_head_fused()
         if not sd["hist"] or (cameras is None and self._small_def_clean()):
-            return None
+            return None if select is None else (None, None)
         order = self.optimizer.small_groups()
         ps, ms, vs = self.optimizer.small_pointers(order)
         hist = sd["hist"][::-1]
@@ -349,15 +356,30 @@
                 flags = sd["blk_flag"] = torch.empty((blk.shape[0],), dtype=torch.uint8, device=blk.device)
             Ks = torch.stack([c.create_k_on_gpu() if getattr(c, "K", None) is None else c.K for c in cameras]).contiguous()
             vm = torch.stack([c.world_view_transform.transpose(0, 1) for c in cameras]).contiguous()
+        head = (_lib.stream(), int(self._xyz.shape[0]), ps, ms, vs, _lib.dptr(pk), _lib.dptr(gk),
+                _lib.dptr(self._row_g_step, torch.int32), _lib.dptr(blk, torch.int32), int(hist[0][0]), nh, lr, sidx,
+                pos_margin, scale_gain, float(b1), float(b2), float(order[0]["eps"]), 1.0 / float(self.args.bsz), C,
+                _lib.dptr(vm, None, True), _lib.dptr(Ks, None, True), int(utils.get_img_width()), int(utils.get_img_height()),
+                0.3, 0.01, 1e10)
+        if fused:
+            from ... import gsplat
+            xyz, rot, sca = self._xyz.detach(), self._rotation.detach(), self._scaling.detach()
+            assert xyz.data_ptr() == ps[0] and sca.data_ptr() == ps[2] and rot.data_ptr() == ps[3], (
+                "the optimizer's small-attribute tensors are not the model's")
+
+            def count(temp, tb, cum):
+                _lib.check(_lib.lib().clmgs_adam_small_deferred_select(
+                    *head, _lib.dptr(flags, torch.uint8), _lib.dptr(rot, torch.float32), float(select["radius_clip"]),
+                    _lib.dptr(temp), tb, _lib.dptr(cum)))
+            sel = gsplat.visibility_select(xyz, rot, sca, vm, Ks, int(utils.get_img_width()), int(utils.get_img_height()),
+                                           radius_clip=float(select["radius_clip"]), block_flags=flags, count=count,
+                                           union32=bool(select.get("union32", False)))
+            return flags, sel
         _lib.check(_lib.lib().clmgs_adam_small_deferred(
-            _lib.stream(), int(self._xyz.shape[0]), ps, ms, vs, _lib.dptr(pk), _lib.dptr(gk),
-            _lib.dptr(self._row_g_step, torch.int32), _lib.dptr(blk, torch.int32), int(hist[0][0]), nh, lr, sidx,
-            pos_margin, scale_gain, float(b1), float(b2), float(order[0]["eps"]), 1.0 / float(self.args.bsz), C,
-            _lib.dptr(vm, None, True), _lib.dptr(Ks, None, True), int(utils.get_img_width()), int(utils.get_img_height()),
-            0.3, 0.01, 1e10, 0 if cameras is not None else 1, _lib.dptr(flags, torch.uint8, True)))
+            *head, 0 if cameras is not None else 1, _lib.dptr(flags, torch.uint8, True)))
         if cameras is None:
             self._small_def_dirty = False
-        return flags
+        return flags if select is None else (flags, None)
 
     def flush_small(self):
         if self.small_deferred:
diff --git a/clm_gs_amd/utils.py b/clm_gs_amd/utils.py
--- a/clm_gs_amd/utils.py
+++ b/clm_gs_amd/utils.py
@@ -47,6 +47,7 @@
         dp_small_max_log_gain=0.7,
         binning="tile",
         deferred_small_adam=True,
+        fused_batch_head=True,
         allocator_reservoir=True,
         split_catch_up=True,
         early_first_catch_up=True,
diff --git a/include/clmgs.h b/include/clmgs.h
--- a/include/clmgs.h
+++ b/include/clmgs.h
@@ -35,6 +35,7 @@
                                          void* temp, size_t temp_bytes, int64_t* cum_totals,
                                          const uint8_t* block_flags);
 int clmgs_visibility_select_emit(void* stream, int C, int N, const void* temp, int64_t* out);
+int clmgs_visibility_select_emit_u32(void* stream, int C, int N, const void* temp, int64_t* out, int32_t* union32);
 int clmgs_projection_bwd(void* stream, int C, int N, const float* means, const float* quats,
                          const float* scales, const float* viewmats, const float* Ks, int width,
                          int height, float eps2d, const int32_t* radii, const float* v_means2d,
@@ -381,6 +382,14 @@
                               double beta2, double eps, float grad_scale, int C, const float* viewmats, const float* Ks,
                               int width, int height, float eps2d, float near_plane, float far_plane, int flush_all,
                               uint8_t* blk_flag );
+int clmgs_adam_small_deferred_select(void* stream, int64_t n, float* const* params, float* const* exp_avg,
+                                     float* const* exp_avg_sq, void* packed_p, const void* packed_g,
+                                     const int32_t* g_stamp, int32_t* blk_last, int to_step, int n_hist,
+                                     const double* lr4_hist, const int32_t* step_index, const float* pos_margin,
+                                     const float* scale_gain, double beta1, double beta2, double eps, float grad_scale,
+                                     int C, const float* viewmats, const float* Ks, int width, int height, float eps2d,
+                                     float near_plane, float far_plane, uint8_t* blk_flag, const float* quats_raw,
+                                     float radius_clip, void* temp, size_t temp_bytes, int64_t* cum_totals);
 
 int clmgs_device_errors(uint32_t* bits, int reset);
 
diff --git a/profiles/make_pmc_json.py b/profiles/make_pmc_json.py
--- a/profiles/make_pmc_json.py
+++ b/profiles/make_pmc_json.py
@@ -13,6 +13,7 @@
     "clmgs_adam_rows": ["adam_rows_kernel"],
     "clmgs_adam_catch_up": ["adam_catch_up"],
     "clmgs_adam_small_deferred": ["adam_small_deferred_kernel"],
+    "clmgs_adam_small_deferred_select": ["adam_small_deferred_kernel<true>"],
     "clmgs_isect3_front": ["isect3_rows_kernel", "isect3_rows_finish_kernel"],
     "clmgs_isect3_bin": ["isect3_tile_scan_kernel", "isect3_scatter_kernel", "isect3_sort_"],
 }
diff --git a/profiles/timeline.py b/profiles/timeline.py
--- a/profiles/timeline.py
+++ b/profiles/timeline.py
@@ -6,7 +6,7 @@
 c = sqlite3.connect(db)
 rows = list(c.execute("select name, start, end, stream_id from kernels order by start"))
 if arg.startswith("step"):
-    marks = [r[1] for r in rows if "visibility_bits" in r[0]]
+    marks = [r[1] for r in rows if "visibility_bits" in r[0] or "adam_small_deferred_kernel<true>" in r[0]]
     k = int(arg[4:] or 2)
     t0, t_end = marks[-k - 1], marks[-k]
     rows = [r for r in rows if t0 <= r[1] < t_end]
diff --git a/profiles/timeline_host.py b/profiles/timeline_host.py
--- a/profiles/timeline_host.py
+++ b/profiles/timeline_host.py
@@ -20,7 +20,7 @@
 t_end = max([k[2] for k in kern] + [x[1] for x in copies])
 t0 = t_end - win if win else min(k[1] for k in kern)
 if arg and arg.startswith("batches"):
-    marks = [k[1] for k in kern if "visibility_bits" in k[0]]
+    marks = [k[1] for k in kern if "visibility_bits" in k[0] or "adam_small_deferred_kernel<true>" in k[0]]
     nb = int(arg[7:] or 2)
     t0, t_end = marks[-nb - 1], marks[-1]
 kern = [k for k in kern if t0 <= k[1] < t_end]
diff --git a/profiles/timeline_streams.py b/profiles/timeline_streams.py
--- a/profiles/timeline_streams.py
+++ b/profiles/timeline_streams.py
@@ -6,7 +6,7 @@
 c = sqlite3.connect(db)
 rows = list(c.execute("select name, start, end, queue_id, grid_x, workgroup_x, lds_size from kernels order by start"))
 if arg.startswith("step"):
-    marks = [r[1] for r in rows if "visibility_bits" in r[0]]
+    marks = [r[1] for r in rows if "visibility_bits" in r[0] or "adam_small_deferred_kernel<true>" in r[0]]
     k = int(arg[4:] or 2)
     t0, t_end = marks[-k - 1], marks[-k]
     rows = [r for r in rows if t0 <= r[1] < t_end]
```

Result: no change. 198.0 (median of 6 runs) (+1.5%).
